# invesalius/invesalius3

Measured on AMD Instinct MI355X. Metric: Mvoxel/s segmentation + Mtriangles/s marching-cubes, 512^3 int16, 1/2/4/8 GPU, higher is better.
Workload: dtype i16; 1 GPU; configs[1]: 512x512x512 int16 per GPU, threshold(226..3071) + 26-neighbour region-grow + marching-cubes(mask@127); global_voxels=134217728, parallelism=z-slab x1, collectives=none, overlap=none

## Files before the change

include/ivx.h:

```cpp
#ifndef IVX_H
#define IVX_H
#include <stddef.h>
#include <stdint.h>

#ifdef __cplusplus
extern "C" {
#endif

#define IVX_OK 0
#define IVX_EINVAL (-1)
#define IVX_ERANGE (-2)
#define IVX_ENOMEM (-3)
#define IVX_EDOM (-4)
#define IVX_EHIP (-5)
#define IVX_ESTALE (-6)

#define IVX_U8 0
#define IVX_I16 1
#define IVX_F64 2
#define IVX_U16 3
#define IVX_F32 4
#define IVX_I32 5
#define IVX_I64 6
#define IVX_I8 7
// ... 307 lines not shown

int ivx_mask_snapshot_header_bytes(int64_t n, size_t *nbytes);
int ivx_dev_mask_snapshot_scan(const uint8_t *src, int64_t n, void *header, int64_t *literal_blocks, void *stream);
int ivx_dev_mask_snapshot_pack(const uint8_t *src, int64_t n, const void *header, void *pool, int64_t literal_blocks, void *stream);
int ivx_dev_mask_snapshot_restore(uint8_t *dst, int64_t n, const void *header, const void *pool, int64_t literal_blocks,
                                  int64_t plane_bytes, uint8_t *plane_flags, void *stream);
int ivx_mask_snapshot(const uint8_t *matrix, size_t nbytes, void **header, void **pool, int64_t *literal_blocks);
int ivx_mask_snapshot_restore(uint8_t *matrix, size_t nbytes, const void *header, const void *pool, int64_t literal_blocks,
                              size_t plane_bytes, int64_t *planes_written);

int ivx_dev_mask_boolean(int op, const uint8_t *m1, const uint8_t *m2, uint8_t *out, int64_t n, void *stream);
int ivx_dev_masked_density_i16(const int16_t *img, const uint8_t *mask, int64_t n, void *acc5, void *stream);
int ivx_mask_boolean(int op, const uint8_t *m1, const int64_t st1[3], const uint8_t *m2, const int64_t st2[3], uint8_t *out,
                     const int64_t sto[3], const int64_t shape[3]);
int ivx_masked_density_i16(const int16_t *img, const int64_t img_strides[3], const uint8_t *mask,
                           const int64_t mask_strides[3], const int64_t shape[3], double *out5);

int ivx_dev_convolve_non_zero(const double *volume, int64_t sz, int64_t sy, int64_t sx, const double *kernel, int64_t skz,
                              int64_t sky, int64_t skx, int cval, double *out, void *stream);
int ivx_mask_area_scratch_bytes(int64_t sz, int64_t sy, int64_t sx, size_t *nbytes);
int ivx_dev_mask_area_u8(const uint8_t *mask, int64_t sz, int64_t sy, int64_t sx, const double *kernel27_dev,
                         double *scratch, double *area_dev, void *stream);
int ivx_convolve_non_zero(const double *volume, const int64_t shape[3], const int64_t vol_strides[3], const double *kernel,
                          const int64_t kshape[3], int cval, double *out);
int ivx_mask_area(const uint8_t *mask, const int64_t shape[3], const int64_t mask_strides[3], const double spacing_xyz[3],
                  double *area);

typedef struct ivx_flood_plan {
    int64_t dz, dy, dx;
    int64_t wx;
    uint32_t strct_bits;
} ivx_flood_plan;
int ivx_flood_bits_bytes(const ivx_flood_plan *p, size_t *nbytes);
int ivx_flood_scratch_bytes(const ivx_flood_plan *p, size_t *nbytes);
int ivx_flood_strct_bits(const uint8_t *strct, const int64_t sshape[3], uint32_t *bits);
int ivx_dev_flood_clear(const ivx_flood_plan *p, uint64_t *reached, void *scratch, void *stream);
int ivx_dev_flood_candidates(const ivx_flood_plan *p, int dtype, const void *data, double t0, double t1,
                             const uint8_t *barrier, int barrier_mode, double fill, uint64_t *cand, void *stream);
int ivx_dev_flood_candidates_ranges(const ivx_flood_plan *p, const int16_t *data, double t0, double t1,
                                    const uint8_t *barrier, int barrier_mode, double fill, const uint32_t *ranges,
                                    uint64_t *cand, void *stream);
int ivx_dev_flood_seed(const ivx_flood_plan *p, int dtype, const void *data, double t0, double t1,
                       const int64_t *seeds_xyz, int64_t nseeds, uint64_t *cand, uint64_t *reached,
                       void *scratch, void *stream);
int ivx_dev_flood_run(const ivx_flood_plan *p, const uint64_t *cand, uint64_t *reached, void *scratch,
                      int *rounds, void *stream);
int ivx_dev_flood_grow(const ivx_flood_plan *p, int dtype, const void *data, double t0, double t1,
                       const int64_t *seeds_xyz, int64_t nseeds, uint64_t *cand, uint64_t *reached, void *scratch,
                       int *rounds, void *stream);
int ivx_dev_flood_visits(const ivx_flood_plan *p, const void *scratch, uint32_t out[2], void *stream);
int ivx_flood_describe(const ivx_flood_plan *p, int64_t nseeds, int32_t out[8]);
int ivx_dev_flood_arm_gate(const void *scratch, uint32_t *word, uint32_t value, uint32_t below_tiles);
int ivx_dev_flood_disarm_gate(const void *scratch);
int ivx_dev_gate_wait(const uint32_t *word, uint32_t value, uint32_t timeout_us, void *stream);
int ivx_dev_gate_open(uint32_t *word, uint32_t value, void *stream);
int ivx_dev_flood_mark_slab(const ivx_flood_plan *p, void *scratch, int64_t z0, int64_t z1, void *stream);
int ivx_dev_bits_combine(uint64_t *dst, const uint64_t *src, int64_t nwords, int op, void *stream);
int ivx_dev_flood_or_plane(const ivx_flood_plan *p, const uint64_t *cand, uint64_t *reached, int64_t z,
                           const uint64_t *plane, void *scratch, int *changed, void *stream);
int ivx_dev_flood_or_planes(const ivx_flood_plan *p, const uint64_t *cand, uint64_t *reached, int64_t z_a,
                            const uint64_t *plane_a, int64_t z_b, const uint64_t *plane_b, void *scratch, int *changed,
                            void *stream);
int ivx_dev_flood_or_planes_dev(const ivx_flood_plan *p, const uint64_t *cand, uint64_t *reached, int64_t z_a,
                                const uint64_t *plane_a, int64_t z_b, const uint64_t *plane_b, void *scratch,
                                uint32_t *changed_dev, void *stream);
int ivx_dev_flood_or_planes_acc(const ivx_flood_plan *p, const uint64_t *cand, uint64_t *reached, int64_t z_a,
                                const uint64_t *plane_a, int64_t z_b, const uint64_t *plane_b, void *scratch,
                                uint32_t *changed_dev, void *stream);
int ivx_dev_flood_apply(const ivx_flood_plan *p, const uint64_t *reached, int dtype, void *target,
                        double fill, void *stream);
int ivx_dev_flood_apply_levels(const ivx_flood_plan *p, const uint64_t *reached, const uint64_t *inside_bits, uint8_t *mask,
                               int v_in, int v_sel, void *stream);
int ivx_dev_mask_from_planes(const ivx_flood_plan *p, const uint64_t *inside_bits, const uint64_t *reached, uint8_t *mask,
                             int v_in, int v_sel, void *stream);
enum { IVX_FLOOD_WRITE_NONE = 0, IVX_FLOOD_WRITE_MASK_FROM_PLANES = 1, IVX_FLOOD_WRITE_APPLY_LEVELS = 2, IVX_FLOOD_WRITE_APPLY_U8 = 3 };
typedef struct ivx_flood_write {
    int32_t kind, v_in, v_sel, reserved;
    const uint64_t *inside_bits;
    uint8_t *mask;
} ivx_flood_write;
int ivx_dev_flood_grow_select(const ivx_flood_plan *p, int dtype, const void *data, double t0, double t1,
                              const int64_t *seeds_xyz, int64_t nseeds, uint64_t *cand, uint64_t *reached, void *scratch,
                              int *rounds, const ivx_flood_write *write, int look_ahead, void *stream);
int ivx_flood_look_ahead(int64_t n_list, int32_t *look_ahead);
int ivx_dev_flood_apply2(const ivx_flood_plan *p, const uint64_t *reached, uint8_t *out, int fill, uint8_t *mask,
                         int select, void *stream);
int ivx_dev_flood_count(const ivx_flood_plan *p, const uint64_t *reached, int64_t *count, void *stream);
int ivx_flood_edges_bytes(const ivx_flood_plan *p, size_t *nbytes);
int ivx_dev_flood_edges_auto(const ivx_flood_plan *p, const int16_t *data, const uint8_t *out, float pfrac, int fill,
                             uint64_t *edges, void *stream);
int ivx_dev_flood_seed_forced(const ivx_flood_plan *p, const int64_t *seeds_xyz, int64_t nseeds, uint64_t *cand,
                              uint64_t *reached, void *scratch, void *stream);
int ivx_dev_flood_run_edges(const ivx_flood_plan *p, const uint64_t *edges, uint64_t *reached, void *scratch, int *rounds,
                            void *stream);
int ivx_floodfill(int dtype, const void *data, const int64_t shape[3], const int64_t strides[3], int64_t x, int64_t y,
                  int64_t z, double v, int fill, uint8_t *out, const int64_t out_strides[3]);
int ivx_floodfill_auto_threshold(const int16_t *data, const int64_t shape[3], const int64_t strides[3],
                                 const int64_t *seeds_xyz, int64_t nseeds, float pfrac, int fill, uint8_t *out,
                                 const int64_t out_strides[3]);
int ivx_dev_jump_flooding(float *dist, int32_t *owners, const int64_t shape[3], const int32_t *sites_host, int64_t nsites,
                          int normalize, void *stream);
int ivx_jump_flooding(float *dist, const int64_t dist_strides[3], int32_t *owners, const int64_t owner_strides[3],
                      const int64_t shape[3], const int32_t *sites, int64_t nsites, int normalize);
int ivx_floodfill_threshold(int dtype, const void *data, const int64_t shape[3], const int64_t strides[3],
                            const int64_t *seeds_xyz, int64_t nseeds, double t0, double t1, int fill,
                            const uint8_t *strct, const int64_t sshape[3], uint8_t *out,
                            const int64_t out_strides[3]);
int ivx_floodfill_threshold_inplace(int dtype, void *data, const int64_t shape[3], const int64_t strides[3],
                                    const int64_t *seeds_xyz, int64_t nseeds, double t0, double t1,
                                    double fill, const uint8_t *strct, const int64_t sshape[3]);

int ivx_dev_fill_holes(uint8_t *mask, const uint32_t *labels, int64_t n, uint32_t nlabels, uint32_t max_size,
                       uint32_t *sizes , int *status2 ,
                       void *stream);
int ivx_fill_holes_automatically(uint8_t *mask, const int64_t shape[3], const int64_t mask_strides[3],
                                 const uint32_t *labels, const int64_t label_strides[3], uint32_t nlabels,
                                 uint32_t max_size, int *modified);
int ivx_dev_fill_holes_auto(uint8_t *mask, int64_t dz, int64_t dy, int64_t dx, const uint8_t *strct, const int64_t sshape[3],
                            uint32_t max_size, int *modified, void *stream);
int ivx_fill_holes_auto(uint8_t *mask, const int64_t shape[3], const int64_t mask_strides[3], const uint8_t *strct,
                        const int64_t sshape[3], uint32_t max_size, int *modified);

int ivx_dev_lut_u16(const int16_t *img, int64_t n, double window, double level, int top255, uint16_t *out,
                    void *stream);
int ivx_dev_lut_i16(const int16_t *img, int64_t n, double window, double level, int top255, int16_t *out,
                    void *stream);
int ivx_dev_shift_min_u16(const int16_t *img, int64_t n, int imin, uint16_t *out, void *stream);
int ivx_dev_morph_gradient_u16(const uint16_t *in, int64_t dz, int64_t dy, int64_t dx, const int size[3],
                               uint16_t *out, void *stream);
int ivx_dev_watershed_merge(uint8_t *mask, const uint8_t *tmp, int64_t n, int overwrite, void *stream);
int ivx_watershed_prepare(const int16_t *img, const int64_t shape[3], const int64_t strides[3], int use_ww_wl,
                          double window, double level, const int gradient_size[3] , uint16_t *out);
int ivx_watershed_merge(uint8_t *mask, const int64_t shape[3], const int64_t mask_strides[3], const uint8_t *tmp,
                        const int64_t tmp_strides[3], int overwrite);

int ivx_dev_sk_cost_levels(const uint16_t *image, int mdtype, const void *markers, int64_t dz, int64_t dy, int64_t dx,
                           const uint8_t strct[27], uint16_t *C, int max_levels, double stop_frac, int *levels_done,
                           int64_t *reached, int64_t *rounds, void *stream);
int ivx_dev_ws_cost_levels(const uint16_t *cost_image, int mdtype, const void *markers, int64_t dz, int64_t dy, int64_t dx,
                           uint16_t *C, int max_levels, double stop_frac, int *levels_done, int64_t *reached,
                           int64_t *rounds, void *stream);
int ivx_dev_watershed_ift(const uint16_t *cost, int mdtype, const void *markers, int64_t dz, int64_t dy, int64_t dx,
                          const uint8_t strct[27], void *out_labels ,
                          uint8_t *out_u8 , uint16_t *cost_out , int64_t stats[16],
                          void *stream);
int ivx_watershed_ift(int idtype , const void *input, const int64_t shape[3], int mdtype,
                      const void *markers, const uint8_t strct[27], void *output, uint16_t *cost_out, int64_t stats[16]);

int ivx_dev_watershed_sk(const uint16_t *image, int mdtype, const void *markers, int64_t dz, int64_t dy, int64_t dx,
                         const uint8_t strct[27], void *out_labels ,
                         int32_t *out_i32 , uint8_t *out_u8 ,
                         uint16_t *cost_out , int64_t stats[16], void *stream);
int ivx_watershed_sk(int idtype , const void *input, const int64_t shape[3], int mdtype,
                     const void *markers, const uint8_t strct[27], int32_t *output, uint16_t *cost_out, int64_t stats[16]);

int ivx_do_watershed(const int16_t *img, const int64_t shape[3], const int64_t strides[3], int mdtype, const void *markers,
                     const uint8_t strct[27], int algorithm, const int gradient_size[3] ,
                     int use_ww_wl, double window, double level, uint8_t *out_u8, int64_t stats[16]);
int ivx_do_watershed_into(const int16_t *img, const int64_t shape[3], const int64_t strides[3], int mk_src_dtype, const void *markers,
                          const int64_t mk_strides[3], int mdtype, const uint8_t strct[27], int algorithm,
                          const int gradient_size[3] , int use_ww_wl, double window, double level,
                          uint8_t *out_u8, const int64_t out_strides[3], int64_t stats[16]);

int ivx_dev_masked_stats_i16(const int16_t *img, const uint8_t *sel, int64_t n, int64_t out3[3], void *stream);
int ivx_dev_or_equal_u8(uint8_t *dst, const uint8_t *src, int64_t n, int value, void *stream);
int ivx_dev_flood_apply_where(uint8_t *dst, const uint8_t *src, int64_t n, int value, int fill, void *stream);
// ... 190 lines not shown
```

invesalius3_amd/_lib.py:

```python
from __future__ import annotations

import ctypes
import os

import numpy as np

_HERE = os.path.dirname(os.path.abspath(__file__))
LIB_PATH = os.environ.get("IVX_LIB_PATH") or os.path.join(_HERE, "libivx.so")

IVX_OK, IVX_EINVAL, IVX_ERANGE, IVX_ENOMEM, IVX_EDOM, IVX_EHIP, IVX_ESTALE = 0, -1, -2, -3, -4, -5, -6
U8, I16, F64, U16, F32, I32, I64, I8 = 0, 1, 2, 3, 4, 5, 6, 7
DT = {np.dtype(np.uint8): U8, np.dtype(np.int16): I16, np.dtype(np.float64): F64, np.dtype(np.uint16): U16, np.dtype(np.float32): F32, np.dtype(np.int32): I32,
      np.dtype(np.int64): I64}
MIP_MAX, MIP_MIN, MIP_MEAN, MIP_SUM = 0, 1, 2, 3

c_i64 = ctypes.c_int64
c_vp = ctypes.c_void_p


class McParams(ctypes.Structure):
    _fields_ = [
        ("dtype", ctypes.c_int32), ("pad_xy", ctypes.c_int32), ("pad_bottom", ctypes.c_int32),
        ("pad_top", ctypes.c_int32), ("vtk_pz", ctypes.c_int32), ("niso", ctypes.c_int32),
        ("nz", c_i64), ("ny", c_i64), ("nx", c_i64), ("roi_start", c_i64),
        ("pad_value", ctypes.c_double), ("spacing", ctypes.c_double * 3), ("iso", ctypes.c_double * 2),
    ]


class FloodPlan(ctypes.Structure):
    _fields_ = [("dz", c_i64), ("dy", c_i64), ("dx", c_i64), ("wx", c_i64), ("strct_bits", ctypes.c_uint32)]


FLOOD_WRITE_NONE, FLOOD_WRITE_MASK_FROM_PLANES, FLOOD_WRITE_APPLY_LEVELS, FLOOD_WRITE_APPLY_U8 = 0, 1, 2, 3


class FloodWrite(ctypes.Structure):
    _fields_ = [("kind", ctypes.c_int32), ("v_in", ctypes.c_int32), ("v_sel", ctypes.c_int32), ("reserved", ctypes.c_int32),
                ("inside_bits", c_vp), ("mask", c_vp)]


class VolrenParams(ctypes.Structure):
    _fields_ = [
        ("width", ctypes.c_int32), ("height", ctypes.c_int32), ("mip", ctypes.c_int32), ("shade", ctypes.c_int32),
        ("skip", ctypes.c_int32), ("n_table", ctypes.c_int32), ("out_u8", ctypes.c_int32), ("clip", ctypes.c_int32),
        ("origin", ctypes.c_double * 3), ("du", ctypes.c_double * 3), ("dv", ctypes.c_double * 3),
        ("dir", ctypes.c_double * 3), ("spacing", ctypes.c_double * 3), ("dt", ctypes.c_double),
        ("ambient", ctypes.c_double), ("diffuse", ctypes.c_double), ("specular", ctypes.c_double),
        ("specular_power", ctypes.c_double), ("background", ctypes.c_double * 3), ("clip_normal", ctypes.c_double * 3),
        ("clip_origin", ctypes.c_double * 3),
    ]


ROI_ELLIPSE, ROI_POLYGON, ROI_MAX_POINTS, ROI_RECORD_BYTES = 0, 1, 2048, 40


class Roi(ctypes.Structure):
    _fields_ = [
        ("image", c_vp), ("row_stride", c_i64), ("elem_stride", c_i64), ("h", c_i64), ("w", c_i64),
        ("kind", ctypes.c_int32), ("n_points", ctypes.c_int32), ("first_point", c_i64),
        ("sx", ctypes.c_double), ("sy", ctypes.c_double), ("cx", ctypes.c_double), ("cy", ctypes.c_double),
        ("a2", ctypes.c_double), ("b2", ctypes.c_double),
        ("x0", c_i64), ("y0", c_i64), ("x1", c_i64), ("y1", c_i64), ("first_block", c_i64), ("n_blocks", c_i64),
    ]


class StaleError(RuntimeError):
    """IVX_ESTALE: a registered host array (resident.bind) was written without a touch; raised only with the stale check on."""


def _declare(lib):
    u64, sz, u64p = ctypes.c_uint64, ctypes.c_size_t, ctypes.POINTER(ctypes.c_uint64)
    i64p = ctypes.POINTER(c_i64)
    for name, args in (("ivx_host_register", [c_vp, sz, u64p]), ("ivx_host_touch", [u64]), ("ivx_host_touch_range", [u64, sz, sz]),
                       ("ivx_host_release", [u64]), ("ivx_host_stats", [u64, u64p]), ("ivx_host_count", [u64p]),
                       ("ivx_host_set_check", [ctypes.c_int]), ("ivx_transfer_stats", [u64p]),
                       ("ivx_upload_strided", [c_vp, c_vp, i64p, i64p, sz]), ("ivx_download_strided", [c_vp, i64p, i64p, c_vp, sz]),
                       ("ivx_image_ranges_bytes", [c_i64, c_i64, c_i64, ctypes.POINTER(sz)]),
                       ("ivx_dev_image_ranges_i16", [c_vp, c_i64, c_i64, c_i64, c_vp, c_vp]),
                       ("ivx_dev_threshold_i16_bits_ranges", [c_vp, c_i64, c_i64, c_i64, ctypes.c_int, ctypes.c_int, c_vp, c_vp, c_vp,
                                                              ctypes.c_int, c_vp]),
                       ("ivx_dev_threshold_i16_plane", [c_vp, c_i64, c_i64, c_i64, ctypes.c_int, ctypes.c_int, c_vp, c_vp]),
                       ("ivx_dev_threshold_i16_plane_ranges", [c_vp, c_i64, c_i64, c_i64, ctypes.c_int, ctypes.c_int, c_vp, c_vp,
                                                               ctypes.c_int, c_vp]),
                       ("ivx_dev_mask_from_planes", [ctypes.POINTER(FloodPlan), c_vp, c_vp, c_vp, ctypes.c_int, ctypes.c_int, c_vp]),
                       ("ivx_dev_flood_candidates_ranges", [ctypes.POINTER(FloodPlan), c_vp, ctypes.c_double, ctypes.c_double, c_vp,
                                                            ctypes.c_int, ctypes.c_double, c_vp, c_vp, c_vp]),
                       ("ivx_dev_flood_grow_select", [ctypes.POINTER(FloodPlan), ctypes.c_int, c_vp, ctypes.c_double, ctypes.c_double,
                                                      c_vp, c_i64, c_vp, c_vp, c_vp, ctypes.POINTER(ctypes.c_int),
                                                      ctypes.POINTER(FloodWrite), ctypes.c_int, c_vp]),
                       ("ivx_flood_look_ahead", [c_i64, ctypes.POINTER(ctypes.c_int32)]),
                       ("ivx_dev_image_flip", [c_vp, c_i64, c_i64, c_i64, sz, ctypes.c_int, c_vp]),
                       ("ivx_image_flip", [c_vp, i64p, i64p, sz, ctypes.c_int]),
                       ("ivx_dev_image_swap_axes", [c_vp, c_i64, c_i64, c_i64, sz, ctypes.c_int, ctypes.c_int, c_vp, c_vp]),
                       ("ivx_image_swap_axes", [c_vp, i64p, i64p, sz, ctypes.c_int, ctypes.c_int, c_vp, i64p]),
                       ("ivx_image_tilt_scratch_bytes", [c_i64, c_i64, c_i64, ctypes.POINTER(sz)]),
                       ("ivx_dev_image_fix_gantry_tilt", [c_vp, c_i64, c_i64, c_i64, c_vp, c_vp, sz, c_vp, c_vp]),
                       ("ivx_image_fix_gantry_tilt", [c_vp, i64p, i64p, c_vp, c_vp]),
                       ("ivx_host_zero", [c_vp, sz]), ("ivx_host_register_zero", [c_vp, sz, u64p]),
                       ("ivx_slice_show_tables_bytes", [ctypes.c_int, ctypes.POINTER(sz)]),
                       ("ivx_dev_slice_show", [c_vp, c_i64, c_i64] * 3 + [c_i64, c_i64, c_vp, c_vp, c_vp, c_vp]),
                       ("ivx_slice_show", [c_vp, c_i64, c_i64] * 3 + [c_i64, c_i64, c_vp, c_vp, c_vp]),
                       ("ivx_mask_snapshot_header_bytes", [c_i64, ctypes.POINTER(sz)]),
                       ("ivx_dev_mask_snapshot_scan", [c_vp, c_i64, c_vp, i64p, c_vp]),
                       ("ivx_dev_mask_snapshot_pack", [c_vp, c_i64, c_vp, c_vp, c_i64, c_vp]),
                       ("ivx_dev_mask_snapshot_restore", [c_vp, c_i64, c_vp, c_vp, c_i64, c_i64, c_vp, c_vp]),
                       ("ivx_mask_snapshot", [c_vp, sz, ctypes.POINTER(c_vp), ctypes.POINTER(c_vp), i64p]),
                       ("ivx_mask_snapshot_restore", [c_vp, sz, c_vp, c_vp, c_i64, sz, i64p]),
                       ("ivx_dev_surface_raster", [c_vp, c_i64, c_vp, c_i64, c_vp, ctypes.c_int, c_vp, c_vp]),
                       ("ivx_dev_surface_resolve", [c_vp, ctypes.c_int, c_vp, ctypes.c_int, c_vp, ctypes.c_int, c_vp, c_vp, c_vp, c_vp]),
                       ("ivx_surface_render", [c_vp, ctypes.c_int, c_vp, ctypes.c_int, c_vp, ctypes.c_int, c_vp, c_vp, c_vp]),
                       ("ivx_dev_roi_density", [c_vp, c_i64, c_vp, c_vp, c_i64, c_vp, c_vp]),
                       ("ivx_roi_density", [c_vp, c_i64, c_vp, c_i64, c_vp]),
                       ("ivx_dev_m3e_filter", [c_i64, c_i64, c_vp, c_vp, c_i64, ctypes.c_int, c_vp, c_vp]),
                       ("ivx_dev_m3e_cut", [c_vp, i64p, i64p, c_vp, ctypes.c_double, c_vp, c_i64, c_i64, c_vp, c_vp, ctypes.c_int, c_vp, c_vp]),
                       ("ivx_dev_m3e_brush_stroke", [c_vp, c_vp, i64p, i64p, c_vp, c_vp, c_vp, c_i64, ctypes.c_double, ctypes.c_int, c_vp,
                                                     c_vp]),
                       ("ivx_dev_m3e_equal", [c_vp, c_vp, c_i64, ctypes.POINTER(ctypes.c_int), c_vp]),
                       ("ivx_dev_m3e_apply", [c_vp, c_vp, i64p, i64p, c_vp, c_vp]),
                       ("ivx_m3e_filter", [c_i64, c_i64, c_vp, c_vp, c_i64, ctypes.c_int, c_vp]),
                       ("ivx_m3e_cut", [c_vp, i64p, i64p, c_vp, ctypes.c_double, c_vp, c_i64, c_i64, c_vp, c_vp, c_i64, c_vp, c_vp,
                                        ctypes.c_int, i64p]),
                       ("ivx_m3e_brush_stroke", [c_vp, c_vp, i64p, i64p, c_vp, c_vp, c_i64, ctypes.c_double, ctypes.c_int, i64p]),
                       ("ivx_m3e_apply", [c_vp, c_vp, i64p, i64p, i64p]), ("ivx_m3e_flag_planes", [c_vp, i64p, i64p])):
        fn = getattr(lib, name)
        fn.argtypes, fn.restype = args, ctypes.c_int


_lib = None


def lib() -> ctypes.CDLL:
    global _lib
    if _lib is None:
        if not os.path.exists(LIB_PATH):
            raise ImportError(
                "libivx.so not found at %s: build it with `python -m invesalius3_amd.build` "
                "(there is no CPU fallback in this package)" % LIB_PATH)
        _lib = ctypes.CDLL(LIB_PATH)
        _lib.ivx_last_error.restype = ctypes.c_char_p
        _declare(_lib)
    return _lib


def last_error() -> str:
    return (lib().ivx_last_error() or b"").decode("utf-8", "replace")


def check(rc: int, what: str = "ivx") -> int:
    if rc >= 0:
        return rc
    msg = "%s: %s" % (what, last_error())
    if rc == IVX_EINVAL:
        raise TypeError(msg)
    if rc == IVX_ERANGE:
        raise IndexError(msg)
    if rc == IVX_ENOMEM:
        raise MemoryError(msg)
    if rc == IVX_EDOM:
        raise ValueError(msg)
    if rc == IVX_ESTALE:
        raise StaleError(msg)
    raise RuntimeError(msg)


def i64(seq):
    return (c_i64 * len(seq))(*[int(v) for v in seq])


def ptr(a: np.ndarray):
    return ctypes.c_void_p(a.ctypes.data)


# ... 60 lines not shown
```

invesalius3_amd/csrc/ivx_internal.h:

```cpp
#pragma once
#include <hip/hip_runtime.h>
#include <stdint.h>
#include <stdio.h>
#include <string.h>

#include "../../include/ivx.h"

namespace ivx {

void set_error(const char *fmt, ...);

#define IVX_HIP(expr)                                                                      \
    do {                                                                                   \
        hipError_t e__ = (expr);                                                           \
        if (e__ != hipSuccess) {                                                           \
            ivx::set_error("%s:%d %s -> %s", __FILE__, __LINE__, #expr, hipGetErrorString(e__)); \
            return e__ == hipErrorOutOfMemory ? IVX_ENOMEM : IVX_EHIP;                     \
        }                                                                                  \
    } while (0)

bool trace_enabled();
#define IVX_LAUNCH_CHECK()                                                                 \
    do {                                                                                   \
        IVX_HIP(hipGetLastError());                                                        \
        if (ivx::trace_enabled()) {                                                        \
            fprintf(stderr, "ivx trace: launched %s:%d ...", __FILE__, __LINE__);          \
            fflush(stderr);                                                                \
            IVX_HIP(hipDeviceSynchronize());                                               \
            fprintf(stderr, " ok\n");                                                      \
        }                                                                                  \
    } while (0)

#define IVX_REQUIRE(cond, code, ...)                                                       \
    do {                                                                                   \
        if (!(cond)) {                                                                     \
            ivx::set_error(__VA_ARGS__);                                                   \
            return (code);                                                                 \
        }                                                                                  \
    } while (0)

static inline hipStream_t S(void *s) { return (hipStream_t)s; }
static inline int64_t cdiv(int64_t a, int64_t b) { return (a + b - 1) / b; }
static inline size_t dtype_size(int dt) {
    switch (dt) {
    case IVX_U8: return 1;
    case IVX_I16: return 2;
    case IVX_U16: return 2;
    case IVX_F64: return 8;
    default: return 0;
    }
}

enum { WS_IN = 0, WS_OUT, WS_AUX0, WS_AUX1, WS_AUX2, WS_AUX3, WS_SMALL, WS_CCL0, WS_CCL1, WS_MCLIST, WS_MCV, WS_MCST, WS_MESH, WS_MESH2, WS_HOLES, WS_LUT, WS_WSIFT, WS_WSSK, WS_WSA, WS_WSLINK, WS_COUNT };
int ws_get(int slot, size_t nbytes, void **dptr);
int ws_get_s(int slot, hipStream_t stream, size_t nbytes, void **dptr);
uint64_t host_epoch();
int ws_release_s(int slot, hipStream_t stream, size_t keep_below);
struct HostCallGuard {
    HostCallGuard();
    ~HostCallGuard();
};
int hs_get(int slot, size_t nbytes, void **hptr);

int copy_h2d(void *dst_dev, const void *src, size_t n);
int copy_d2h(void *dst, const void *src_dev, size_t n);

int upload_strided(void *dst_dev, const void *src, const int64_t shape[3], const int64_t strides[3], size_t isz,
                   int hslot);
int download_strided(void *dst, const int64_t shape[3], const int64_t strides[3], const void *src_dev, size_t isz,
                     int hslot);
int download_strided2(void *dst, const int64_t shape[2], const int64_t strides[2], const void *src_dev, size_t isz,
                      int hslot);
int mirror_host_view(const void *view, const int64_t shape[3], const int64_t strides[3], size_t isz, void *d_scratch, int hslot);

struct MirrorHold;
int mirror_acquire(const void *p, size_t n, bool reads, MirrorHold **hold, void **mirror);
int mirror_fetch(MirrorHold *hold, void *host, const void *mirror, size_t n);
void mirror_release(MirrorHold *hold, size_t written);

void ccl_forget_stream(void *stream);
void ccl_invalidate(const void *scratch);
int ccl_small_components(const ivx_flood_plan *p, const uint64_t *cand, uint64_t *out, uint32_t max_size, int *any_small,
                         const void *scratch_key, hipStream_t st);
bool ccl_supported(uint32_t strct_bits);
int ccl_run(const ivx_flood_plan *p, const uint64_t *cand, uint64_t *reached, const void *scratch_key, hipStream_t st);
enum FloodMode {
    FLOOD_SYMMETRIC,
    FLOOD_DIRECTED,
    FLOOD_LINEAR,
};
int flood_run(const ivx_flood_plan *p, const uint64_t *planes, FloodMode mode, uint64_t *reached, void *scratch, int *rounds,
              void *stream);

int mailbox_publish(const void *dsrc, int ndwords, hipStream_t st, uint32_t *seq_out);
int mailbox_wait(uint32_t seq, hipStream_t st, uint32_t *out, int ndwords);
int mailbox_reserve(uint32_t **slot_out, uint32_t *seq_out);
int mailbox_wait_reserved(uint32_t seq, hipStream_t st, uint32_t *out, int ndwords, int *got);
int vote_publish(int32_t *votes, hipStream_t st, uint32_t *seq_out);
int progress_line(hipStream_t stream, volatile unsigned long long **line, uint32_t *tag);
void progress_forget_stream(void *stream);

}
```

invesalius3_amd/csrc/k_flood.hip:

```cpp
#include <math.h>
#include <map>
#include <mutex>
#include <stdlib.h>

#include "flood_tiles.h"
#include "words_from_records.h"

namespace {

constexpr int NT = TY * TZ;
constexpr int HY = TY + 2, HZ = TZ + 2;
constexpr int BATCH = 8;
constexpr int SUB = 1;
constexpr unsigned int CLOSED = 0x40u;

template <typename T> __device__ __forceinline__ double as_double(T v) { return (double)v; }

template <typename T, int BAR>
__global__ __launch_bounds__(256) void k_flood_candidates16(const short8_t *__restrict__ data,
                                                            const uint4 *__restrict__ bar, int64_t nchunks, double t0,
                                                            double t1, double fill, uint16_t *__restrict__ cand) {
    const int64_t stride = (int64_t)gridDim.x * blockDim.x;
    const int lo = (int)ceil(t0 < -70000.0 ? -70000.0 : t0), hi = (int)floor(t1 > 70000.0 ? 70000.0 : t1);
    const unsigned fb = (unsigned)(uint8_t)fill;
    for (int64_t c = (int64_t)blockIdx.x * blockDim.x + threadIdx.x; c < nchunks; c += stride) {
        const short8_t a = __builtin_nontemporal_load(&data[2 * c]);
        const short8_t b = __builtin_nontemporal_load(&data[2 * c + 1]);
        uint4 q = make_uint4(0, 0, 0, 0);
        if (BAR == 1) q = bar[c];
        const unsigned bw[4] = {q.x, q.y, q.z, q.w};
        unsigned m = 0;
#pragma unroll
        for (int e = 0; e < 16; e++) {
            const int v = (int)(T)(e < 8 ? a[e & 7] : b[e & 7]);
            bool ok = v >= lo && v <= hi;
            if (BAR == 1) ok = ok && ((bw[e >> 2] >> (8 * (e & 3))) & 0xffu) != fb;
            if (BAR == 2) ok = ok && (double)v != fill;
            m |= ok ? (1u << e) : 0u;
        }
        cand[c] = (uint16_t)m;
    }
}

__global__ __launch_bounds__(256) void k_flood_candidates_words(const short8_t *__restrict__ data, const unsigned *__restrict__ ranges,
                                                                int64_t nwords, double t0, double t1,
                                                                unsigned long long *__restrict__ cand) {
    const int lo = (int)ceil(t0 < -70000.0 ? -70000.0 : t0), hi = (int)floor(t1 > 70000.0 ? 70000.0 : t1);
    words_from_records(data, ranges, nwords, lo, hi, cand);
}

__global__ __launch_bounds__(256) void k_flood_candidates16_ranges(const short8_t *__restrict__ data,
                                                                   const uint4 *__restrict__ bar,
                                                                   const unsigned *__restrict__ ranges, int64_t nchunks,
                                                                   double t0, double t1, double fill,
                                                                   uint16_t *__restrict__ cand) {
    const int64_t stride = (int64_t)gridDim.x * blockDim.x;
    const int lo = (int)ceil(t0 < -70000.0 ? -70000.0 : t0), hi = (int)floor(t1 > 70000.0 ? 70000.0 : t1);
    const unsigned fb = (unsigned)(uint8_t)fill;
    int64_t c = (int64_t)blockIdx.x * blockDim.x + threadIdx.x;
    if (c >= nchunks) return;
    unsigned rec = ranges[c >> 2];
    for (;;) {
        const int64_t cn = c + stride;
        unsigned rec_next = 0;
        if (cn < nchunks) rec_next = ranges[cn >> 2];
        const int mn = (int)(short)(rec & 0xffffu), mx = (int)(short)(rec >> 16);
        unsigned m = 0;
        if (!(mx < lo || mn > hi)) {
            const bool inside = mn >= lo && mx <= hi;
            if (inside) {
                m = 0xffffu;
            } else {
                const short8_t a = __builtin_nontemporal_load(&data[2 * c]);
                const short8_t b = __builtin_nontemporal_load(&data[2 * c + 1]);
#pragma unroll
                for (int e = 0; e < 16; e++) {
                    const int v = (int)(e < 8 ? a[e & 7] : b[e & 7]);
                    m |= (v >= lo && v <= hi) ? (1u << e) : 0u;
                }
            }
            if (m) {
                const uint4 q = bar[c];
                const unsigned bw[4] = {q.x, q.y, q.z, q.w};
#pragma unroll
                for (int e = 0; e < 16; e++)
                    if (((bw[e >> 2] >> (8 * (e & 3))) & 0xffu) == fb) m &= ~(1u << e);
            }
        }
        cand[c] = (uint16_t)m;
// ... 813 lines not shown
                if (!ok[d]) continue;
                const int64_t n = base + x + off[d];
                const int nv = data[n];
                if (out[n] != fill && nv >= t0 && nv <= t1) m[d] |= 1u << e;
            }
        }
        const int64_t plane = total;
#pragma unroll
        for (int d = 0; d < 6; d++) edges[d * plane + i] = (uint8_t)m[d];
    }
}

__global__ void k_flood_seed_forced(Tiles t, const int64_t *__restrict__ seeds, int64_t nseeds,
                                    unsigned long long *__restrict__ cand, unsigned long long *__restrict__ reached,
                                    uint8_t *__restrict__ dirty) {
    const int64_t n = (int64_t)blockIdx.x * blockDim.x + threadIdx.x;
    if (n >= nseeds) return;
    const int64_t x = seeds[3 * n], y = seeds[3 * n + 1], z = seeds[3 * n + 2];
    const int64_t w = (z * t.dy + y) * t.wx + (x >> 6);
    const unsigned long long bit = 1ull << (x & 63);
    if (cand) atomicOr(&cand[w], bit);
    atomicOr(&reached[w], bit);
    mark_tile_nbhd(t, dirty, z / TZ, y / TY, x >> 6);
}

template <typename T>
__global__ __launch_bounds__(256) void k_flood_apply(Tiles t, const uint8_t *__restrict__ reached, T *__restrict__ out,
                                                     T fill) {
    const int64_t bpr = t.wx * 8;
    const int64_t total = t.dz * t.dy * bpr;
    const int64_t stride = (int64_t)gridDim.x * blockDim.x;
    const bool aligned8 = ((uintptr_t)out & 7) == 0 && (t.dx & 7) == 0;
    for (int64_t i = (int64_t)blockIdx.x * blockDim.x + threadIdx.x; i < total; i += stride) {
        const unsigned m = reached[i];
        if (!m) continue;
        const int64_t row = i / bpr, q = i - row * bpr;
        T *o = out + row * t.dx + q * 8;
        if (sizeof(T) == 1 && m == 0xffu && aligned8) {
            *reinterpret_cast<unsigned long long *>(o) = 0x0101010101010101ull * (unsigned long long)(uint8_t)fill;
            continue;
        }
#pragma unroll
        for (int e = 0; e < 8; e++)
            if (m >> e & 1u) o[e] = fill;
    }
}

__global__ __launch_bounds__(256) void k_flood_apply16(const uint16_t *__restrict__ reached, int64_t nchunks,
                                                       uint4 *__restrict__ out, uint8_t fill) {
    const int64_t stride = (int64_t)gridDim.x * 1024;
    const unsigned int f4 = 0x01010101u * fill;
    for (int64_t i0 = (int64_t)blockIdx.x * 1024 + threadIdx.x; i0 < nchunks; i0 += stride) {
        unsigned int m[4];
        uint4 o[4];
#pragma unroll
        for (int u = 0; u < 4; u++) {
            const int64_t i = i0 + u * 256;
            m[u] = i < nchunks ? reached[i] : 0u;
            o[u] = make_uint4(0u, 0u, 0u, 0u);
        }
#pragma unroll
        for (int u = 0; u < 4; u++)
            if (m[u] && m[u] != 0xffffu) o[u] = out[i0 + u * 256];
#pragma unroll
        for (int u = 0; u < 4; u++) {
            if (!m[u]) continue;
            uint4 v = make_uint4(f4, f4, f4, f4);
            if (m[u] != 0xffffu) {
                auto blend = [&](unsigned int old, unsigned int bits4) {
                    const unsigned int sel = ((bits4 & 1u) * 0xffu) | ((bits4 >> 1 & 1u) * 0xff00u) |
                                             ((bits4 >> 2 & 1u) * 0xff0000u) | ((bits4 >> 3 & 1u) * 0xff000000u);
                    return (old & ~sel) | (f4 & sel);
                };
                v.x = blend(o[u].x, m[u] & 15u);
                v.y = blend(o[u].y, m[u] >> 4 & 15u);
                v.z = blend(o[u].z, m[u] >> 8 & 15u);
                v.w = blend(o[u].w, m[u] >> 12 & 15u);
            }
            out[i0 + u * 256] = v;
        }
    }
}

struct ApplyWhen {
    const unsigned int *next_len;
    unsigned long long *line;
    unsigned long long report;
};
template <bool ALL>
__global__ __launch_bounds__(256) void k_flood_apply_levels16(const uint16_t *__restrict__ reached, const uint16_t *__restrict__ inside,
                                                              int64_t nchunks, uint4 *__restrict__ out, uint8_t v_in, uint8_t v_sel,
                                                              ApplyWhen when) {
    if (when.next_len) {
        if (*when.next_len != 0u) return;
        if (blockIdx.x == 0 && threadIdx.x == 0) __hip_atomic_store(&when.line[2], when.report, __ATOMIC_RELAXED, __HIP_MEMORY_SCOPE_SYSTEM);
    }
    const int64_t stride = (int64_t)gridDim.x * 1024;
    const unsigned int in4 = 0x01010101u * v_in, sel4 = 0x01010101u * v_sel;
    for (int64_t i0 = (int64_t)blockIdx.x * 1024 + threadIdx.x; i0 < nchunks; i0 += stride) {
        unsigned int m[4], b[4];
#pragma unroll
        for (int u = 0; u < 4; u++) {
            const int64_t i = i0 + u * 256;
            m[u] = i < nchunks && (!ALL || reached) ? reached[i] : 0u;
            b[u] = i < nchunks ? inside[i] : 0u;
        }
#pragma unroll
        for (int u = 0; u < 4; u++) {
            if (ALL ? i0 + u * 256 >= nchunks : !m[u]) continue;
            auto bytes = [](unsigned int bits4) { return ((bits4 * 0x00204081u) & 0x01010101u) * 0xffu; };
            auto word = [&](unsigned int r4, unsigned int i4) {
                const unsigned int rs = bytes(r4);
                return (sel4 & rs) | (in4 & bytes(i4) & ~rs);
            };
            out[i0 + u * 256] = make_uint4(word(m[u] & 15u, b[u] & 15u), word(m[u] >> 4 & 15u, b[u] >> 4 & 15u),
                                           word(m[u] >> 8 & 15u, b[u] >> 8 & 15u), word(m[u] >> 12 & 15u, b[u] >> 12 & 15u));
        }
    }
}

__global__ __launch_bounds__(256) void k_flood_apply2(Tiles t, const uint8_t *__restrict__ reached, uint8_t *__restrict__ out,
                                                      uint8_t fill, uint8_t *__restrict__ mask, uint8_t select) {
    const int64_t bpr = t.wx * 8;
    const int64_t total = t.dz * t.dy * bpr;
    const int64_t stride = (int64_t)gridDim.x * blockDim.x;
    const bool aligned8 = (((uintptr_t)out | (uintptr_t)mask) & 7) == 0;
    for (int64_t i = (int64_t)blockIdx.x * blockDim.x + threadIdx.x; i < total; i += stride) {
        const unsigned m = reached[i];
        if (!m) continue;
        const int64_t row = i / bpr, q = i - row * bpr;
        const int64_t base = row * t.dx + q * 8;
        if (m == 0xffu && ((t.dx & 7) == 0) && aligned8) {
            *reinterpret_cast<unsigned long long *>(out + base) = 0x0101010101010101ull * fill;
            *reinterpret_cast<unsigned long long *>(mask + base) = 0x0101010101010101ull * select;
            continue;
        }
#pragma unroll
        for (int e = 0; e < 8; e++)
            if (m >> e & 1u) {
                out[base + e] = fill;
                mask[base + e] = select;
            }
    }
}

__global__ __launch_bounds__(256) void k_flood_count(const unsigned long long *__restrict__ bits, int64_t nwords,
                                                     unsigned long long *__restrict__ total) {
    unsigned long long s = 0;
    const int64_t stride = (int64_t)gridDim.x * blockDim.x;
    for (int64_t i = (int64_t)blockIdx.x * blockDim.x + threadIdx.x; i < nwords; i += stride) s += __popcll(bits[i]);
#pragma unroll
    for (int o = 32; o > 0; o >>= 1) s += __shfl_xor(s, o, 64);
    if ((threadIdx.x & 63) == 0 && s) atomicAdd(total, s);
}

static inline int grid_for(int64_t n) {
    const int64_t b = ivx::cdiv(n, 256);
    return (int)(b < 1 ? 1 : (b < 32768 ? b : 32768));
}

template <typename T>
static int run_candidates(const Tiles &t, const void *data, double t0, double t1, const uint8_t *bar, int bar_mode,
                          double fill, uint8_t *cand, hipStream_t st) {
    const int64_t total = t.dz * t.dy * t.wx * 8;
    if (!total) return IVX_OK;
    if (sizeof(T) == 2 && t.dx % 64 == 0 && (((uintptr_t)data | (uintptr_t)bar | (uintptr_t)cand) & 15) == 0) {
        const int64_t nchunks = t.dz * t.dy * t.dx / 16;
        const int64_t blocks = ivx::cdiv(nchunks, 256);
        const int gg = (int)(blocks < 16384 ? blocks : 16384);
        const short8_t *d8 = (const short8_t *)data;
        const uint4 *b4 = (const uint4 *)bar;
        uint16_t *c16 = (uint16_t *)cand;
        if (bar_mode == 0) hipLaunchKernelGGL((k_flood_candidates16<T, 0>), dim3(gg), dim3(256), 0, st, d8, b4, nchunks, t0, t1, fill, c16);
        else if (bar_mode == 1) hipLaunchKernelGGL((k_flood_candidates16<T, 1>), dim3(gg), dim3(256), 0, st, d8, b4, nchunks, t0, t1, fill, c16);
        else hipLaunchKernelGGL((k_flood_candidates16<T, 2>), dim3(gg), dim3(256), 0, st, d8, b4, nchunks, t0, t1, fill, c16);
        IVX_LAUNCH_CHECK();
        return IVX_OK;
    }
    const int g = grid_for(total);
    if (bar_mode == 0)
        hipLaunchKernelGGL((k_flood_candidates<T, 0>), dim3(g), dim3(256), 0, st, (const T *)data, bar, t, t0, t1, fill, cand);
    else if (bar_mode == 1)
        hipLaunchKernelGGL((k_flood_candidates<T, 1>), dim3(g), dim3(256), 0, st, (const T *)data, bar, t, t0, t1, fill, cand);
    else
        hipLaunchKernelGGL((k_flood_candidates<T, 2>), dim3(g), dim3(256), 0, st, (const T *)data, bar, t, t0, t1, fill, cand);
    IVX_LAUNCH_CHECK();
    return IVX_OK;
}

}

extern "C" int ivx_flood_bits_bytes(const ivx_flood_plan *p, size_t *nbytes) {
    Tiles t;
    int rc = make_tiles(p, &t);
    if (rc) return rc;
    *nbytes = al256((size_t)(t.dz * t.dy * t.wx) * 8);
    return IVX_OK;
}

extern "C" int ivx_flood_scratch_bytes(const ivx_flood_plan *p, size_t *nbytes) {
// ... 183 lines not shown
        return e && !strcmp(e, "ccl");
    }();
    return ccl;
}
static bool coarse_ok(const Tiles &t, ivx::FloodMode mode) {
    static const bool coarse_on = [] {
        const char *e = getenv("IVX_FLOOD_COARSE");
        return !(e && e[0] == '0');
    }();
    return coarse_on && mode == ivx::FLOOD_SYMMETRIC && t.conn != 0 && t.wx <= 64 && (t.nty + 2) * (t.ntz + 2) <= CROWS_MAX &&
           t.nty * t.ntz <= (int64_t)CT * CRP;
}
static Blocks coarse_blocks(const Tiles &t) {
    static const int bxs_env = [] {
        const char *e = getenv("IVX_FLOOD_BLOCK");
        return e ? atoi(e) : 0;
    }();
    Blocks bk;
    bk.bxs = 16;
    while (bk.bxs < 64 && ((64 / bk.bxs) * t.wx > 64 || bk.bxs < bxs_env)) bk.bxs *= 2;
    bk.q = 64 / bk.bxs;
    return bk;
}
static int coarse_lanes(const Tiles &t) {
    int ct = 64;
    while (ct < CT && ct < t.nty * t.ntz) ct *= 2;
    return ct;
}
template <bool FRESH>
static int coarse_pass(const Tiles &t, const FScratch &s, char *scr, const uint64_t *cand, uint64_t *reached, const Fresh &f,
                       int ncnt, hipStream_t st) {
    const Blocks bk = coarse_blocks(t);
    uint8_t *dirty0 = (uint8_t *)(scr + s.off_dirty0), *dirty1 = (uint8_t *)(scr + s.off_dirty1);
    unsigned int *cnt = (unsigned int *)(scr + s.off_cnt), *list0 = (unsigned int *)(scr + s.off_list0);
    unsigned long long *rowF = (unsigned long long *)(scr + s.off_full), *rowW = (unsigned long long *)(scr + s.off_whole);
    unsigned int *seed_ok = (unsigned int *)(scr + s.off_status) + 8;
    const unsigned groups = (unsigned)(t.nty * t.ntz);
    const int ct = coarse_lanes(t);
    hipLaunchKernelGGL(k_flood_block_flags<FRESH>, dim3(groups), dim3(256), 0, st, t, bk, (unsigned long long *)cand,
                       (const unsigned long long *)reached, dirty0, dirty1, rowF, rowW, cnt, ncnt, f.sp, f.dtype, f.data, f.t0,
                       f.t1, seed_ok);
    IVX_LAUNCH_CHECK();
    auto coarse = t.conn == 26 ? k_flood_coarse<26, FRESH> : t.conn == 18 ? k_flood_coarse<18, FRESH> : k_flood_coarse<6, FRESH>;
    hipLaunchKernelGGL(coarse, dim3(1), dim3(ct), 0, st, t, bk, (const unsigned long long *)rowF, rowW, f.sp,
                       (const unsigned int *)seed_ok);
    IVX_LAUNCH_CHECK();
    hipLaunchKernelGGL(k_flood_block_apply<FRESH>, dim3(groups), dim3(256), 0, st, t, bk, (const unsigned long long *)cand,
                       (unsigned long long *)reached, (const unsigned long long *)rowW, dirty0, list0, cnt, f.sp,
                       (const unsigned int *)seed_ok);
    IVX_LAUNCH_CHECK();
    return IVX_OK;
}
static unsigned round_grid_cap(const Tiles &t) { return (unsigned)(t.ntiles < 1536 ? t.ntiles : 1536); }
template <typename Done>
static int poll_line(volatile unsigned long long *line, long spins, hipStream_t st, Done done, const char *never,
                     unsigned long long *word) {
    for (long n = 0; n < spins; n++) {
        *word = __atomic_load_n((const unsigned long long *)line, __ATOMIC_ACQUIRE);
        if (done(*word)) return IVX_OK;
#if defined(__x86_64__)
        __builtin_ia32_pause();
#endif
    }
    IVX_HIP(hipStreamSynchronize(st));
    *word = __atomic_load_n((const unsigned long long *)line, __ATOMIC_ACQUIRE);
    IVX_REQUIRE(done(*word), IVX_EHIP, "%s", never);
    return IVX_OK;
}
static int levels_check(const Tiles &t, const uint64_t *reached, const uint64_t *inside_bits, const uint8_t *mask, int v_in, int v_sel,
                        bool all) {
    if (all) {
        IVX_REQUIRE(inside_bits && mask, IVX_EINVAL, "mask_from_planes: null plane or mask");
        IVX_REQUIRE(t.dx % 64 == 0 && ((uintptr_t)mask & 15) == 0 && (((uintptr_t)inside_bits | (uintptr_t)reached) & 7) == 0, IVX_EINVAL,
                    "mask_from_planes: rows of whole 64-voxel words, a 16-byte aligned mask and 8-byte aligned planes only");
        IVX_REQUIRE(v_in >= 0 && v_in <= 255 && v_sel >= 0 && v_sel <= 255, IVX_EINVAL, "mask_from_planes: levels are bytes");
    } else {
        IVX_REQUIRE(reached && inside_bits && mask, IVX_EINVAL, "flood_apply_levels: null plane or mask");
        IVX_REQUIRE(t.dx % 64 == 0 && ((uintptr_t)mask & 15) == 0, IVX_EINVAL,
                    "flood_apply_levels: rows of whole 64-voxel words and a 16-byte aligned mask only");
        IVX_REQUIRE(v_in >= 0 && v_in <= 255 && v_sel >= 0 && v_sel <= 255, IVX_EINVAL, "flood_apply_levels: levels are bytes");
    }
    return IVX_OK;
}
static int launch_levels(const Tiles &t, const uint64_t *reached, const uint64_t *inside, uint8_t *mask, int v_in, int v_sel, bool all,
                         const ApplyWhen &when, hipStream_t st) {
    const int64_t nchunks = t.dz * t.dy * t.dx / 16;
    if (!nchunks) return IVX_OK;
    const int64_t blocks = ivx::cdiv(nchunks, 1024);
    auto k = all ? k_flood_apply_levels16<true> : k_flood_apply_levels16<false>;
    hipLaunchKernelGGL(k, dim3((unsigned)(blocks < 16384 ? blocks : 16384)), dim3(256), 0, st, (const uint16_t *)reached,
                       (const uint16_t *)inside, nchunks, (uint4 *)mask, (uint8_t)v_in, (uint8_t)v_sel, when);
    IVX_LAUNCH_CHECK();
    return IVX_OK;
}
constexpr unsigned AHEAD_LONG_LIST = 384u;
static int default_look_ahead(unsigned n_list) { return n_list >= AHEAD_LONG_LIST ? 0 : 1; }
struct EarlyWrite {
    const ivx_flood_write *w;
    bool written;
};
constexpr unsigned EARLY_BELOW = 96u;
constexpr int EARLY_TRIES = 2;
static int flood_run_impl(const ivx_flood_plan *p, const uint64_t *cand, ivx::FloodMode mode, uint64_t *reached, void *scratch_,
                          int *rounds, void *stream, const Fresh *fresh = nullptr, int look_ahead = -1, EarlyWrite *early = nullptr) {
    const bool sym = mode == ivx::FLOOD_SYMMETRIC;
    Tiles t;
    int rc = make_tiles(p, &t);
    if (rc) return rc;
    if (rounds) *rounds = 0;
    hipStream_t st = ivx::S(stream);
    GateArm arm = {nullptr, 0u, 0u};
    {
        std::lock_guard<std::mutex> lk(g_gates_mu);
        auto it = g_gates.find(scratch_);
        if (it != g_gates.end()) {
            arm = it->second;
            g_gates.erase(it);
        }
    }
    struct GateGuard {
        GateArm &a;
        hipStream_t st;
        ~GateGuard() {
            if (a.word) hipLaunchKernelGGL(k_gate_set, dim3(1), dim3(64), 0, st, a.word, a.value);
        }
    } gate_guard = {arm, st};
    if (t.ntiles == 0) return IVX_OK;
    const FScratch s = make_fscratch(t);
    char *scr = (char *)scratch_;
    uint8_t *dirty[2] = {(uint8_t *)(scr + s.off_dirty0), (uint8_t *)(scr + s.off_dirty1)};
    unsigned int *cnt = (unsigned int *)(scr + s.off_cnt);
    constexpr int CCL_ESCAPE_ROUNDS = 48;
    if (sym && flood_mode_ccl() && ivx::ccl_supported(p->strct_bits)) {
        if (rounds) *rounds = 1;
        IVX_HIP(hipMemsetAsync(dirty[0], 0, (size_t)t.ntiles, st));
        return ivx::ccl_run(p, cand, reached, scratch_, st);
    }
    int total_rounds = 0;
    unsigned int *list[2] = {(unsigned int *)(scr + s.off_list0), (unsigned int *)(scr + s.off_list1)};
    constexpr int RING = 2 * BATCH;
    static const int env_ahead = [] {
        const char *e = getenv("IVX_FLOOD_BATCH");
        if (!e || !*e) return -1;
        const int v = atoi(e);
        return v < 0 ? 0 : (v > BATCH ? BATCH : v);
    }();
    const int fixed_ahead = env_ahead >= 0 ? env_ahead : (look_ahead > BATCH ? BATCH : look_ahead);
    int ahead = fixed_ahead >= 0 ? fixed_ahead : 1;
    if (coarse_ok(t, mode)) {
        static const Fresh no_seeds = {0, nullptr, 0.0, 0.0, {{}, 0}};
        rc = fresh ? coarse_pass<true>(t, s, scr, cand, reached, *fresh, CNT_CLEARED, st)
                   : coarse_pass<false>(t, s, scr, cand, reached, no_seeds, CNT_CLEARED, st);
        if (rc) return rc;
    } else {
        IVX_REQUIRE(!fresh, IVX_EINVAL, "flood: the fused start needs the coarse pass");
        IVX_HIP(hipMemsetAsync(cnt, 0, CNT_CLEARED * 4, st));
        hipLaunchKernelGGL(k_flood_build_list, dim3((unsigned)ivx::cdiv(t.ntiles, 256)), dim3(256), 0, st, t, dirty[0], list[0], cnt);
        IVX_LAUNCH_CHECK();
    }
    volatile unsigned long long *line = nullptr;
    uint32_t tag = 0;
    if ((rc = ivx::progress_line(st, &line, &tag))) return rc;
    const unsigned grid_max = round_grid_cap(t);
    unsigned grid = grid_max;
    int64_t queued = 0;
    auto round_kernel = mode == ivx::FLOOD_LINEAR ? k_flood_round_list<2> : mode == ivx::FLOOD_DIRECTED ? k_flood_round_list<1> : k_flood_round_list<0>;
    auto queue_round = [&]() -> int {
        const int r = (int)(queued % RING), cur = (int)(queued & 1);
        const unsigned int tr = (unsigned int)(tag << 24) | (unsigned int)((queued + 1) & 0xffffff);
        hipLaunchKernelGGL(round_kernel, dim3(grid), dim3(NT), 0, st, t, (const unsigned long long *)cand,
                           (unsigned long long *)reached, (const unsigned int *)list[cur], (const unsigned int *)(cnt + r), dirty[cur],
                           dirty[cur ^ 1], list[cur ^ 1], cnt + (r + 1) % RING, cnt + (r + 2) % RING, cnt,
                           (unsigned long long *)line, tr,
                           arm.word, arm.value, arm.below);
        IVX_LAUNCH_CHECK();
        queued++;
        return IVX_OK;
    };
    static const bool trace = getenv("IVX_FLOOD_TRACE") != nullptr;
    static const bool early_on = [] {
        const char *e = getenv("IVX_FLOOD_EARLY");
        return !(e && e[0] == '0');
    }();
    const bool early_all = early && early->w->kind == IVX_FLOOD_WRITE_MASK_FROM_PLANES;
    int early_left = 0;
    if (early_on && early && (early_all || early->w->kind == IVX_FLOOD_WRITE_APPLY_LEVELS) &&
        levels_check(t, reached, early->w->inside_bits, early->w->mask, early->w->v_in, early->w->v_sel, early_all) == IVX_OK)
        early_left = EARLY_TRIES;
    if (early_left) __atomic_store_n((unsigned long long *)line + 2, 0ull, __ATOMIC_RELEASE);
    int64_t early_at = -1;
    unsigned long long early_report = 0;
    bool early_seen = false;
    unsigned int prev_list = 0xffffffffu;
    int64_t seen = 0;
    for (;;) {
        while (queued < seen + 1 + ahead)
            if ((rc = queue_round())) return rc;
        unsigned long long v = 0;
        rc = poll_line(line, 20000000L, st,
                       [&](unsigned long long w) {
                           if (early_at >= 0 && __atomic_load_n((const unsigned long long *)line + 2, __ATOMIC_ACQUIRE) == early_report)
                               return early_seen = true;
                           return (uint32_t)(w >> 56) == tag && (int64_t)((w >> 32) & 0xffffffull) > seen;
                       },
                       "flood: the queued rounds never reported", &v);
        if (rc) return rc;
        if (early_seen) {
            const unsigned long long u = __atomic_load_n((const unsigned long long *)line + 1, __ATOMIC_ACQUIRE);
            total_rounds = (uint32_t)(u >> 56) == tag ? (int)((u >> 32) & 0xffffffull) : 0;
            early->written = true;
            if (trace) fprintf(stderr, "ivx flood: the write behind round %lld went ahead (%d rounds with work)\n", (long long)early_at, total_rounds);
            break;
        }
        seen = (int64_t)((v >> 32) & 0xffffffull);
        const unsigned int n_list = (unsigned int)(v & 0xffffffffull);
        if (trace) fprintf(stderr, "ivx flood: round %lld starts with %u of %lld tiles (%lld queued)\n", (long long)seen, n_list,
                           (long long)t.ntiles, (long long)queued);
        if (n_list < arm.below) arm.word = nullptr;
        grid = n_list >= 384u ? grid_max : (n_list >= 96u ? (grid_max < 512u ? grid_max : 512u) : (grid_max < 128u ? grid_max : 128u));
        if (fixed_ahead < 0) ahead = default_look_ahead(n_list);
        if (n_list == 0) {
            const unsigned long long u = __atomic_load_n((const unsigned long long *)line + 1, __ATOMIC_ACQUIRE);
            total_rounds = (uint32_t)(u >> 56) == tag ? (int)((u >> 32) & 0xffffffull) : 0;
            if (early_at >= 0 && total_rounds <= early_at) early->written = true;
            break;
        }
        if (early_at >= 0 && seen > early_at) early_at = -1;
        if (early_left > 0 && early_at < 0 && n_list < EARLY_BELOW && n_list <= prev_list / 2u) {
            early_at = queued;
            early_left--;
            early_report = ((unsigned long long)tag << 56) | ((unsigned long long)(queued & 0xffffff) << 32) | 1ull;
            if (trace) fprintf(stderr, "ivx flood: write queued behind round %lld\n", (long long)queued);
            rc = launch_levels(t, reached, early->w->inside_bits, early->w->mask, early->w->v_in, early->w->v_sel, early_all,
                               ApplyWhen{cnt + queued % RING, (unsigned long long *)line, early_report}, st);
            if (rc) return rc;
        }
        prev_list = n_list;
        total_rounds = (int)seen;
        if (sym && total_rounds >= CCL_ESCAPE_ROUNDS && ivx::ccl_supported(p->strct_bits)) {
            IVX_HIP(hipMemsetAsync(dirty[0], 0, (size_t)t.ntiles, st));
            IVX_HIP(hipMemsetAsync(dirty[1], 0, (size_t)t.ntiles, st));
            if ((rc = ivx::ccl_run(p, cand, reached, scratch_, st))) return rc;
            total_rounds += 1;
            break;
        }
        IVX_REQUIRE(total_rounds < (1 << 24) - 64, IVX_EHIP, "flood: did not converge");
    }
    if (rounds) *rounds = total_rounds;
    return IVX_OK;
}

constexpr int AHEAD_CHAINED = 3;
int ivx::flood_run(const ivx_flood_plan *p, const uint64_t *planes, ivx::FloodMode mode, uint64_t *reached, void *scratch,
                   int *rounds, void *stream) {
    return flood_run_impl(p, planes, mode, reached, scratch, rounds, stream, nullptr, AHEAD_CHAINED);
}

extern "C" int ivx_dev_flood_run(const ivx_flood_plan *p, const uint64_t *cand, uint64_t *reached, void *scratch_,
                                 int *rounds, void *stream) {
    return flood_run_impl(p, cand, ivx::FLOOD_SYMMETRIC, reached, scratch_, rounds, stream, nullptr, AHEAD_CHAINED);
}
static bool fused_start(const Tiles &t, int64_t nseeds) {
    static const bool fused_on = [] {
        const char *e = getenv("IVX_FLOOD_FUSED");
        return !(e && e[0] == '0');
    }();
    return fused_on && nseeds >= 1 && nseeds <= 16 && t.ntiles > 0 && !flood_mode_ccl() && coarse_ok(t, ivx::FLOOD_SYMMETRIC);
}
static int flood_grow_impl(const ivx_flood_plan *p, int dtype, const void *data, double t0, double t1, const int64_t *seeds_xyz,
                           int64_t nseeds, uint64_t *cand, uint64_t *reached, void *scratch_, int *rounds, void *stream,
                           int look_ahead, EarlyWrite *early = nullptr) {
    Tiles t;
    int rc = make_tiles(p, &t);
    if (rc) return rc;
    IVX_REQUIRE(ivx::dtype_size(dtype), IVX_EINVAL, "flood: unsupported dtype %d", dtype);
    for (int64_t n = 0; n < nseeds; n++) {
        const int64_t x = seeds_xyz[3 * n], y = seeds_xyz[3 * n + 1], z = seeds_xyz[3 * n + 2];
        IVX_REQUIRE(x >= 0 && y >= 0 && z >= 0 && x < t.dx && y < t.dy && z < t.dz, IVX_ERANGE,
                    "flood: seed (%lld,%lld,%lld) outside volume (%lld,%lld,%lld) [x,y,z]", (long long)x, (long long)y,
                    (long long)z, (long long)t.dx, (long long)t.dy, (long long)t.dz);
    }
    if (!fused_start(t, nseeds)) {
        if ((rc = ivx_dev_flood_clear(p, reached, scratch_, stream))) return rc;
        if ((rc = ivx_dev_flood_seed(p, dtype, data, t0, t1, seeds_xyz, nseeds, cand, reached, scratch_, stream))) return rc;
        return flood_run_impl(p, cand, ivx::FLOOD_SYMMETRIC, reached, scratch_, rounds, stream, nullptr, look_ahead, early);
    }
    ivx::ccl_invalidate(scratch_);
    Fresh f;
    f.dtype = dtype;
    f.data = data;
    f.t0 = t0;
    f.t1 = t1;
    f.sp.n = (int)nseeds;
    for (int64_t n = 0; n < nseeds; n++)
        for (int q = 0; q < 3; q++) f.sp.xyz[n][q] = seeds_xyz[3 * n + q];
    return flood_run_impl(p, cand, ivx::FLOOD_SYMMETRIC, reached, scratch_, rounds, stream, &f, look_ahead, early);
}
extern "C" int ivx_dev_flood_grow(const ivx_flood_plan *p, int dtype, const void *data, double t0, double t1,
                                  const int64_t *seeds_xyz, int64_t nseeds, uint64_t *cand, uint64_t *reached, void *scratch_,
                                  int *rounds, void *stream) {
    return flood_grow_impl(p, dtype, data, t0, t1, seeds_xyz, nseeds, cand, reached, scratch_, rounds, stream, AHEAD_CHAINED);
}
extern "C" int ivx_flood_look_ahead(int64_t n_list, int32_t *look_ahead) {
    IVX_REQUIRE(look_ahead && n_list >= 0, IVX_EINVAL, "flood_look_ahead: NULL or negative argument");
    *look_ahead = default_look_ahead(n_list > 0xffffffffll ? 0xffffffffu : (unsigned)n_list);
    return IVX_OK;
}
extern "C" int ivx_dev_flood_visits(const ivx_flood_plan *p, const void *scratch_, uint32_t out[2], void *stream) {
    IVX_REQUIRE(scratch_ && out, IVX_EINVAL, "flood_visits: NULL argument");
    Tiles t;
    int rc = make_tiles(p, &t);
    if (rc) return rc;
    out[0] = out[1] = 0u;
    if (t.ntiles == 0) return IVX_OK;
    const FScratch s = make_fscratch(t);
    hipStream_t st = ivx::S(stream);
    unsigned int w[CNT_CLEARED - STATS_AT];
    IVX_HIP(hipMemcpyAsync(w, (const char *)scratch_ + s.off_cnt + STATS_AT * 4, sizeof w, hipMemcpyDeviceToHost, st));
    IVX_HIP(hipStreamSynchronize(st));
    out[0] = w[0];
    for (int k = 0; k < HIST; k++) out[0] += w[HIST_AT - STATS_AT + k];
    out[1] = w[HIST_AT - STATS_AT];
    return IVX_OK;
}
extern "C" int ivx_flood_describe(const ivx_flood_plan *p, int64_t nseeds, int32_t out[8]) {
    IVX_REQUIRE(out, IVX_EINVAL, "flood_describe: NULL argument");
// ... 78 lines not shown
    return IVX_OK;
}
extern "C" int ivx_dev_flood_disarm_gate(const void *scratch) {
    std::lock_guard<std::mutex> lk(g_gates_mu);
    g_gates.erase(scratch);
    return IVX_OK;
}
extern "C" int ivx_dev_gate_open(uint32_t *word, uint32_t value, void *stream) {
    IVX_REQUIRE(word, IVX_EINVAL, "gate_open: NULL argument");
    hipLaunchKernelGGL(k_gate_set, dim3(1), dim3(64), 0, ivx::S(stream), word, value);
    IVX_LAUNCH_CHECK();
    return IVX_OK;
}
extern "C" int ivx_dev_gate_wait(const uint32_t *word, uint32_t value, uint32_t timeout_us, void *stream) {
    IVX_REQUIRE(word, IVX_EINVAL, "gate_wait: NULL argument");
    hipLaunchKernelGGL(k_gate_wait, dim3(1), dim3(64), 0, ivx::S(stream), word, value, (unsigned long long)timeout_us * 100ull);
    IVX_LAUNCH_CHECK();
    return IVX_OK;
}

extern "C" int ivx_dev_flood_mark_slab(const ivx_flood_plan *p, void *scratch_, int64_t z0, int64_t z1, void *stream) {
    Tiles t;
    int rc = make_tiles(p, &t);
    if (rc) return rc;
    if (z0 < 0) z0 = 0;
    if (z1 > t.dz) z1 = t.dz;
    if (z1 <= z0 || t.ntiles == 0) return IVX_OK;
    const FScratch s = make_fscratch(t);
    const int64_t tz0 = z0 / TZ, tz1 = ivx::cdiv(z1, TZ);
    const int64_t n = (tz1 - tz0) * t.nty * t.wx;
    hipLaunchKernelGGL(k_flood_mark, dim3((unsigned)ivx::cdiv(n, 256)), dim3(256), 0, ivx::S(stream), t, tz0, tz1,
                       (uint8_t *)((char *)scratch_ + s.off_dirty0));
    IVX_LAUNCH_CHECK();
    return IVX_OK;
}

extern "C" int ivx_dev_flood_apply(const ivx_flood_plan *p, const uint64_t *reached, int dtype, void *target,
                                   double fill, void *stream) {
    Tiles t;
    int rc = make_tiles(p, &t);
    if (rc) return rc;
    const int64_t total = t.dz * t.dy * t.wx * 8;
    if (!total) return IVX_OK;
    const int g = grid_for(total);
    hipStream_t st = ivx::S(stream);
    const uint8_t *r = (const uint8_t *)reached;
    if (dtype == IVX_U8 && t.dx % 64 == 0 && ((uintptr_t)target & 15) == 0) {
        const int64_t nchunks = t.dz * t.dy * t.dx / 16;
        const int64_t blocks = ivx::cdiv(nchunks, 1024);
        hipLaunchKernelGGL(k_flood_apply16, dim3((unsigned)(blocks < 16384 ? blocks : 16384)), dim3(256), 0, st,
                           (const uint16_t *)reached, nchunks, (uint4 *)target, (uint8_t)fill);
        IVX_LAUNCH_CHECK();
        return IVX_OK;
    }
    switch (dtype) {
    case IVX_U8: hipLaunchKernelGGL(k_flood_apply<uint8_t>, dim3(g), dim3(256), 0, st, t, r, (uint8_t *)target, (uint8_t)fill); break;
    case IVX_I16: hipLaunchKernelGGL(k_flood_apply<int16_t>, dim3(g), dim3(256), 0, st, t, r, (int16_t *)target, (int16_t)fill); break;
    case IVX_U16: hipLaunchKernelGGL(k_flood_apply<uint16_t>, dim3(g), dim3(256), 0, st, t, r, (uint16_t *)target, (uint16_t)fill); break;
    case IVX_F64: hipLaunchKernelGGL(k_flood_apply<double>, dim3(g), dim3(256), 0, st, t, r, (double *)target, fill); break;
    default: ivx::set_error("flood: unsupported dtype %d", dtype); return IVX_EINVAL;
    }
    IVX_LAUNCH_CHECK();
    return IVX_OK;
}

extern "C" int ivx_dev_flood_apply_levels(const ivx_flood_plan *p, const uint64_t *reached, const uint64_t *inside_bits, uint8_t *mask,
                                          int v_in, int v_sel, void *stream) {
    Tiles t;
    int rc = make_tiles(p, &t);
    if (rc) return rc;
    if ((rc = levels_check(t, reached, inside_bits, mask, v_in, v_sel, false))) return rc;
    return launch_levels(t, reached, inside_bits, mask, v_in, v_sel, false, ApplyWhen{nullptr, nullptr, 0ull}, ivx::S(stream));
}

extern "C" int ivx_dev_mask_from_planes(const ivx_flood_plan *p, const uint64_t *inside_bits, const uint64_t *reached, uint8_t *mask,
                                        int v_in, int v_sel, void *stream) {
    Tiles t;
    int rc = make_tiles(p, &t);
    if (rc) return rc;
    if ((rc = levels_check(t, reached, inside_bits, mask, v_in, v_sel, true))) return rc;
    return launch_levels(t, reached, inside_bits, mask, v_in, v_sel, true, ApplyWhen{nullptr, nullptr, 0ull}, ivx::S(stream));
}

extern "C" int ivx_dev_flood_grow_select(const ivx_flood_plan *p, int dtype, const void *data, double t0, double t1,
                                         const int64_t *seeds_xyz, int64_t nseeds, uint64_t *cand, uint64_t *reached,
                                         void *scratch_, int *rounds, const ivx_flood_write *write, int look_ahead, void *stream) {
    IVX_REQUIRE(write && write->kind >= IVX_FLOOD_WRITE_NONE && write->kind <= IVX_FLOOD_WRITE_APPLY_U8, IVX_EINVAL,
                "flood_grow_select: no write description, or one of an unknown kind");
    IVX_REQUIRE(write->kind == IVX_FLOOD_WRITE_NONE || write->mask, IVX_EINVAL, "flood_grow_select: the write has no mask");
    EarlyWrite early = {write, false};
    int rc = flood_grow_impl(p, dtype, data, t0, t1, seeds_xyz, nseeds, cand, reached, scratch_, rounds, stream, look_ahead, &early);
    if (rc || early.written) return rc;
    switch (write->kind) {
    case IVX_FLOOD_WRITE_MASK_FROM_PLANES:
        return ivx_dev_mask_from_planes(p, write->inside_bits, reached, write->mask, write->v_in, write->v_sel, stream);
    case IVX_FLOOD_WRITE_APPLY_LEVELS:
        return ivx_dev_flood_apply_levels(p, reached, write->inside_bits, write->mask, write->v_in, write->v_sel, stream);
    case IVX_FLOOD_WRITE_APPLY_U8: return ivx_dev_flood_apply(p, reached, IVX_U8, write->mask, (double)write->v_sel, stream);
    default: return IVX_OK;
    }
}

extern "C" int ivx_dev_flood_apply2(const ivx_flood_plan *p, const uint64_t *reached, uint8_t *out, int fill,
                                    uint8_t *mask, int select, void *stream) {
    Tiles t;
    int rc = make_tiles(p, &t);
    if (rc) return rc;
    const int64_t total = t.dz * t.dy * t.wx * 8;
    if (!total) return IVX_OK;
    hipLaunchKernelGGL(k_flood_apply2, dim3(grid_for(total)), dim3(256), 0, ivx::S(stream), t, (const uint8_t *)reached, out,
                       (uint8_t)fill, mask, (uint8_t)select);
    IVX_LAUNCH_CHECK();
    return IVX_OK;
}

extern "C" int ivx_dev_flood_count(const ivx_flood_plan *p, const uint64_t *reached, int64_t *count, void *stream) {
    Tiles t;
    int rc = make_tiles(p, &t);
    if (rc) return rc;
    *count = 0;
    const int64_t nw = t.dz * t.dy * t.wx;
    if (!nw) return IVX_OK;
    void *d_tot;
    if ((rc = ivx::ws_get_s(ivx::WS_SMALL, ivx::S(stream), 64, &d_tot))) return rc;
    hipStream_t st = ivx::S(stream);
    IVX_HIP(hipMemsetAsync(d_tot, 0, 8, st));
    hipLaunchKernelGGL(k_flood_count, dim3(grid_for(nw)), dim3(256), 0, st, (const unsigned long long *)reached, nw,
                       (unsigned long long *)d_tot);
    IVX_LAUNCH_CHECK();
    unsigned long long h = 0;
    IVX_HIP(hipMemcpyAsync(&h, d_tot, 8, hipMemcpyDeviceToHost, st));
    IVX_HIP(hipStreamSynchronize(st));
    *count = (int64_t)h;
    return IVX_OK;
}

template <bool MARK>
__global__ __launch_bounds__(256) void k_flood_or_plane(unsigned long long *__restrict__ dst,
                                                        const unsigned long long *__restrict__ src,
                                                        const unsigned long long *__restrict__ cand, int64_t nwords,
                                                        unsigned int *__restrict__ changed, Tiles t, int64_t z,
                                                        uint8_t *__restrict__ dirty) {
    const int64_t i = (int64_t)blockIdx.x * blockDim.x + threadIdx.x;
    if (i >= nwords) return;
    const unsigned long long add = src[i] & cand[i] & ~dst[i];
    if (add) {
        dst[i] |= add;
        atomicAdd(changed, 1u);
        if (MARK) {
            const int64_t y = i / t.wx, txi = i - y * t.wx;
            mark_tile_nbhd(t, dirty, z / TZ, y / TY, txi);
        }
    }
}

__global__ __launch_bounds__(256) void k_bits_combine(unsigned long long *__restrict__ dst,
                                                      const unsigned long long *__restrict__ src, int64_t n, int op) {
    const int64_t stride = (int64_t)gridDim.x * blockDim.x;
    for (int64_t i = (int64_t)blockIdx.x * blockDim.x + threadIdx.x; i < n; i += stride)
        dst[i] = op == 0 ? (dst[i] | src[i]) : (dst[i] & ~src[i]);
}
extern "C" int ivx_dev_bits_combine(uint64_t *dst, const uint64_t *src, int64_t nwords, int op, void *stream) {
    IVX_REQUIRE(nwords >= 0 && (op == 0 || op == 1), IVX_EINVAL, "bits_combine: bad arguments");
    if (nwords == 0) return IVX_OK;
    const int64_t blocks = ivx::cdiv(nwords, 256);
    hipLaunchKernelGGL(k_bits_combine, dim3((unsigned)(blocks < 8192 ? blocks : 8192)), dim3(256), 0, ivx::S(stream),
                       (unsigned long long *)dst, (const unsigned long long *)src, nwords, op);
    IVX_LAUNCH_CHECK();
    return IVX_OK;
}

extern "C" int ivx_dev_flood_or_plane(const ivx_flood_plan *p, const uint64_t *cand, uint64_t *reached, int64_t z,
                                      const uint64_t *plane, void *scratch_, int *changed, void *stream) {
    Tiles t;
    int rc = make_tiles(p, &t);
    if (rc) return rc;
    IVX_REQUIRE(z >= 0 && z < t.dz, IVX_ERANGE, "flood: plane %lld outside slab", (long long)z);
    const FScratch s = make_fscratch(t);
    const int64_t nw = t.dy * t.wx;
    *changed = 0;
    if (!nw) return IVX_OK;
    hipStream_t st = ivx::S(stream);
    unsigned int *d_chg = (unsigned int *)((char *)scratch_ + s.off_status);
// ... 223 lines not shown
```

invesalius3_amd/csrc/k_mc.hip:

```cpp
#include <algorithm>

#include "mc_common.h"

#define MC_TABLE_QUAL static __device__ __attribute__((aligned(16))) const
#include "../../include/ivx_mc_tables.h"

typedef short short8_t __attribute__((ext_vector_type(8)));
typedef unsigned char uchar16_t __attribute__((ext_vector_type(16)));

using namespace ivx;

namespace {

template <typename T, int NISO>
__global__ __launch_bounds__(256) void k_mc_bits(const T *__restrict__ a, int64_t nrows_src, int64_t nx, int64_t ws,
                                                 double iso0, double iso1, uint8_t *__restrict__ bits0,
                                                 uint8_t *__restrict__ bits1) {
    constexpr int V = 16 / sizeof(T);
    constexpr int OB = V / 8;
    const int64_t cpr = ws * 64 / V;
    const int64_t total = nrows_src * cpr;
    const int64_t stride = (int64_t)gridDim.x * blockDim.x;
    const bool vec = (nx % V == 0) && (((uintptr_t)a & 15) == 0);
    if (vec && ws * 64 == nx) {
        const int64_t nchunk = nrows_src * (nx / V);
        typedef T vec_t __attribute__((ext_vector_type(V)));
        const vec_t *src = reinterpret_cast<const vec_t *>(a);
        for (int64_t t0 = ((int64_t)blockIdx.x * blockDim.x) * 4 + threadIdx.x; t0 < nchunk; t0 += stride * 4) {
            vec_t x[4];
#pragma unroll
            for (int u = 0; u < 4; u++) {
                const int64_t t = t0 + (int64_t)u * blockDim.x;
                if (t < nchunk) x[u] = __builtin_nontemporal_load(&src[t]);
            }
#pragma unroll
            for (int u = 0; u < 4; u++) {
                const int64_t t = t0 + (int64_t)u * blockDim.x;
                if (t >= nchunk) continue;
                unsigned m0 = 0, m1 = 0;
#pragma unroll
                for (int e = 0; e < V; e++) {
                    const double d = (double)(T)x[u][e];
                    m0 |= d >= iso0 ? (1u << e) : 0u;
                    if (NISO == 2) m1 |= d >= iso1 ? (1u << e) : 0u;
                }
                if (OB == 1) {
                    bits0[t] = (uint8_t)m0;
                    if (NISO == 2) bits1[t] = (uint8_t)m1;
                } else {
                    reinterpret_cast<uint16_t *>(bits0)[t] = (uint16_t)m0;
                    if (NISO == 2) reinterpret_cast<uint16_t *>(bits1)[t] = (uint16_t)m1;
                }
            }
        }
        return;
    }
    for (int64_t t = (int64_t)blockIdx.x * blockDim.x + threadIdx.x; t < total; t += stride) {
        const int64_t row = t / cpr, q = t - row * cpr;
        const int64_t x0 = q * V;
        unsigned m0 = 0, m1 = 0;
        if (x0 < nx) {
            const T *r = a + row * nx + x0;
            T v[V];
            if (vec) {
                if (sizeof(T) == 2) {
                    const short8_t c = *reinterpret_cast<const short8_t *>(r);
#pragma unroll
                    for (int e = 0; e < V; e++) v[e] = (T)c[e % 8];
                } else {
                    const uchar16_t c = *reinterpret_cast<const uchar16_t *>(r);
#pragma unroll
                    for (int e = 0; e < V; e++) v[e] = (T)c[e % 16];
                }
            } else {
#pragma unroll
                for (int e = 0; e < V; e++) v[e] = (x0 + e < nx) ? r[e] : (T)0;
            }
#pragma unroll
            for (int e = 0; e < V; e++) {
                const bool valid = vec || (x0 + e < nx);
                const double d = (double)v[e];
                m0 |= (valid && d >= iso0) ? (1u << e) : 0u;
                if (NISO == 2) m1 |= (valid && d >= iso1) ? (1u << e) : 0u;
            }
// ... 32 lines not shown
    const uint64_t exist = mc_lowbits(NX32 - w32 * 64);
    uint64_t srcm = exist;
    if (g.pxy && w32 == 0) srcm &= ~1ull;
    srcm &= mc_lowbits(g.pxy + nx32 - w32 * 64);
    const int32_t x1 = (w32 + 1) * 64;
    const bool exist1 = x1 < NX32;
    const bool src1 = x1 - g.pxy < nx32;
    const int32_t wc = w32 >= ws32 ? (ws32 > 0 ? ws32 - 1 : 0) : w32;
    const int32_t wm = w32 - 1 >= ws32 ? (ws32 > 0 ? ws32 - 1 : 0) : (w32 - 1 < 0 ? 0 : w32 - 1);
    const int32_t wp = w32 + 1 >= ws32 ? (ws32 > 0 ? ws32 - 1 : 0) : w32 + 1;
    const int32_t ja0 = ((int32_t)g.NY - 1 - (int32_t)j) - g.pxy, ka0 = (int32_t)k - g.pb;
    const bool inner = ja0 - 1 >= 0 && ja0 < (int32_t)g.ny && ka0 >= 0 && ka0 + 1 < (int32_t)g.nz;
    if (__all(inner)) {
        const uint64_t padlo = pbits & exist & ~srcm;
        const bool use1 = exist1 && src1;
        const uint32_t nbpad = exist1 ? (uint32_t)pbits & 1u : 0u;
        const uint64_t *row = bits + (uint64_t)((uint32_t)ka0 * (uint32_t)g.ny + (uint32_t)ja0) * (uint64_t)(uint32_t)ws32;
        const uint64_t *pc = row + wc, *pa = row + (g.pxy ? wm : wp);
        const int64_t dj = -g.ws, dk = g.ny * g.ws;
        uint64_t a0[4], a1[4];
#pragma unroll
        for (int q = 0; q < 4; q++) {
            const int64_t d = ((q & 1) ? dj : 0) + ((q >> 1) ? dk : 0);
            a0[q] = pc[d];
            a1[q] = pa[d];
        }
#pragma unroll
        for (int q = 0; q < 4; q++) {
            uint64_t v0;
            uint32_t raw1;
            if (g.pxy) {
                v0 = mc_shl1(a0[q], (uint32_t)(a1[q] >> 32));
                raw1 = (uint32_t)(a0[q] >> 63);
            } else {
                v0 = a0[q];
                raw1 = (uint32_t)a1[q] & 1u;
            }
            const uint64_t lo = (v0 & srcm) | padlo;
            r.c[2 * q] = lo;
            r.c[2 * q + 1] = mc_shr1(lo, use1 ? raw1 : nbpad);
        }
    } else {
        const bool has_m = w32 - 1 >= 0 && w32 - 1 < ws32, has_c = w32 < ws32, has_p = w32 + 1 < ws32;
        uint64_t a0[4], a1[4];
        bool rin[4];
#pragma unroll
        for (int q = 0; q < 4; q++) {
            const int64_t ja = (g.NY - 1 - (j + (q & 1))) - g.pxy, ka = k + (q >> 1) - g.pb;
            rin[q] = ja >= 0 && ja < g.ny && ka >= 0 && ka < g.nz;
            const uint64_t *row = bits + (clampi(ka, g.nz) * g.ny + clampi(ja, g.ny)) * g.ws;
            a0[q] = row[wc];
            a1[q] = g.pxy ? row[wm] : row[wp];
        }
#pragma unroll
        for (int q = 0; q < 4; q++) {
            const uint64_t sc = (rin[q] && has_c) ? a0[q] : 0ull;
            uint64_t v0, raw1;
            if (g.pxy) {
                const uint64_t sm = (rin[q] && has_m) ? a1[q] : 0ull;
                v0 = (sc << 1) | (sm >> 63);
                raw1 = sc >> 63;
            } else {
                const uint64_t sp = (rin[q] && has_p) ? a1[q] : 0ull;
                v0 = sc;
                raw1 = sp & 1ull;
            }
            const uint64_t src = rin[q] ? srcm : 0ull;
            const uint64_t lo = (v0 & src) | (pbits & exist & ~src);
            const uint64_t nb = exist1 ? ((rin[q] && src1) ? raw1 : (pbits & 1ull)) : 0ull;
            r.c[2 * q] = lo;
            r.c[2 * q + 1] = (lo >> 1) | (nb << 63);
        }
    }
    uint64_t any = 0, all = ~0ull;
#pragma unroll
    for (int c = 0; c < 8; c++) {
        any |= r.c[c];
        all &= r.c[c];
    }
    r.active = any & ~all & mc_lowbits(NX32 - 1 - w32 * 64);
    return r;
}

__global__ __launch_bounds__(256) void k_mc_count(const uint64_t *__restrict__ bits, Geom g, size_t nwords,
                                                  uint64_t pbits, uint16_t *__restrict__ counts,
                                                  uint32_t *__restrict__ bsum) {
    __shared__ uint32_t s_part[4], s_wcnt[4];
    __shared__ uint8_t s_ntri[256];
    __shared__ uint64_t s_c[256][5];
    __shared__ uint8_t s_hi[256];
    __shared__ uint16_t s_slot[256];
    const int tid = threadIdx.x, lane = tid & 63, wv = tid >> 6;
    const uint8_t ntri = MC_NTRI[tid];
    const size_t wid = (size_t)blockIdx.x * 256 + tid;
    uint64_t act = 0;
    Corner8 r;
    if (wid < nwords) {
        uint32_t k, j, w;
        mc_split_wid(g, (uint32_t)wid, k, j, w);
        r = load_corners(bits, g, (int64_t)k, (int64_t)j, (int64_t)w, pbits);
        act = r.active;
        if (!act) counts[wid] = 0;
    }
    const unsigned long long am = __ballot(act != 0);
    if (lane == 0) s_wcnt[wv] = (uint32_t)__popcll(am);
    s_ntri[tid] = ntri;
    __syncthreads();
    uint32_t before = 0;
    for (int q = 0; q < wv; q++) before += s_wcnt[q];
    const uint32_t nact = s_wcnt[0] + s_wcnt[1] + s_wcnt[2] + s_wcnt[3];
    if (!nact) {
        if (tid == 0) bsum[blockIdx.x] = 0;
        return;
    }
    if (act) {
        const uint32_t slot = before + (uint32_t)__popcll(am & ((1ull << lane) - 1ull));
        s_slot[slot] = (uint16_t)tid;
        uint32_t hi = 0;
#pragma unroll
        for (int q = 0; q < 4; q++) {
            s_c[slot][q] = r.c[2 * q];
            hi |= (uint32_t)(r.c[2 * q + 1] >> 63) << q;
        }
        s_c[slot][4] = act;
        s_hi[slot] = (uint8_t)hi;
    }
    __syncthreads();
    uint32_t n = 0;
    if ((uint32_t)tid < nact) {
        const uint64_t c0 = s_c[tid][0], c1 = s_c[tid][1], c2 = s_c[tid][2], c3 = s_c[tid][3];
        uint64_t a2 = s_c[tid][4];
        const uint32_t hi = s_hi[tid];
        while (a2) {
            const int b = __builtin_ctzll(a2);
            a2 &= a2 - 1;
            int idx;
            if (b != 63)
                idx = (int)((c0 >> b) & 3ull) | ((int)((c1 >> b) & 3ull) << 2) | ((int)((c2 >> b) & 3ull) << 4) | ((int)((c3 >> b) & 3ull) << 6);
            else
                idx = (int)(c0 >> 63) | ((int)(hi & 1u) << 1) | ((int)(c1 >> 63) << 2) | ((int)(hi >> 1 & 1u) << 3) | ((int)(c2 >> 63) << 4) |
                      ((int)(hi >> 2 & 1u) << 5) | ((int)(c3 >> 63) << 6) | ((int)(hi >> 3 & 1u) << 7);
            n += s_ntri[idx];
        }
        counts[(size_t)blockIdx.x * 256 + s_slot[tid]] = (uint16_t)n;
    }
    uint32_t s = n;
#pragma unroll
    for (int o = 32; o > 0; o >>= 1) s += __shfl_xor(s, o, 64);
    if (lane == 0) s_part[wv] = s;
    __syncthreads();
    if (tid == 0) bsum[blockIdx.x] = s_part[0] + s_part[1] + s_part[2] + s_part[3];
}

__global__ __launch_bounds__(1024) void k_mc_scan(const uint32_t *__restrict__ bsum, size_t n,
                                                  uint64_t *__restrict__ boff, uint32_t *mb, uint32_t seq) {
    __shared__ uint64_t s_wave[16];
    __shared__ uint64_t s_carry;
    __shared__ uint32_t s_tot[64], s_exc[64];
    constexpr int RND = 4;
    const int lane = threadIdx.x & 63, wv = threadIdx.x >> 6;
    const size_t base = (size_t)blockIdx.x * (1024 * 4 * RND);
    uint64_t pre = 0;
    {
        const uint4 *b4 = reinterpret_cast<const uint4 *>(bsum);
        const size_t n4 = base / 4;
        uint64_t p0 = 0, p1 = 0, p2 = 0, p3 = 0;
        size_t i = threadIdx.x;
        for (; i + 3 * 1024 < n4; i += 4 * 1024) {
            const uint4 a = b4[i], b = b4[i + 1024], c = b4[i + 2048], d = b4[i + 3072];
            p0 += (uint64_t)a.x + a.y + a.z + a.w;
            p1 += (uint64_t)b.x + b.y + b.z + b.w;
            p2 += (uint64_t)c.x + c.y + c.z + c.w;
            p3 += (uint64_t)d.x + d.y + d.z + d.w;
        }
        for (; i < n4; i += 1024) {
            const uint4 a = b4[i];
            p0 += (uint64_t)a.x + a.y + a.z + a.w;
        }
        pre = p0 + p1 + p2 + p3;
    }
#pragma unroll
    for (int o = 32; o > 0; o >>= 1) pre += __shfl_xor(pre, o, 64);
    if (lane == 0) s_wave[wv] = pre;
    const bool al16 = ((uintptr_t)bsum & 15) == 0 && ((uintptr_t)boff & 15) == 0;
    uint32_t v[RND][4], inc[RND];
#pragma unroll
    for (int r = 0; r < RND; r++) {
        const size_t i0 = base + (size_t)r * 4096 + (size_t)threadIdx.x * 4;
        if (al16 && i0 + 3 < n) {
            const uint4 a = *reinterpret_cast<const uint4 *>(bsum + i0);
            v[r][0] = a.x; v[r][1] = a.y; v[r][2] = a.z; v[r][3] = a.w;
        } else {
#pragma unroll
            for (int q = 0; q < 4; q++) v[r][q] = i0 + q < n ? bsum[i0 + q] : 0u;
        }
    }
#pragma unroll
    for (int r = 0; r < RND; r++) {
        inc[r] = v[r][0] + v[r][1] + v[r][2] + v[r][3];
#pragma unroll
        for (int o = 1; o < 64; o <<= 1) {
            const uint32_t t = __shfl_up(inc[r], o, 64);
            if (lane >= o) inc[r] += t;
        }
        if (lane == 63) s_tot[r * 16 + wv] = inc[r];
    }
    __syncthreads();
    if (wv == 0) {
        const uint32_t t = s_tot[lane];
        uint32_t e = t;
#pragma unroll
        for (int o = 1; o < 64; o <<= 1) {
            const uint32_t u = __shfl_up(e, o, 64);
            if (lane >= o) e += u;
        }
        s_exc[lane] = e - t;
        uint64_t c = 0;
        for (int q = 0; q < 16; q++) c += s_wave[q];
        if (lane == 0) s_carry = c;
        if (lane == 63 && base + 1024 * 4 * RND >= n) {
            const uint64_t total = c + e;
            boff[n] = total;
            if (mb) {
                mb[0] = (uint32_t)total;
                mb[1] = (uint32_t)(total >> 32);
                __threadfence_system();
                __hip_atomic_store(&mb[63], seq, __ATOMIC_RELEASE, __HIP_MEMORY_SCOPE_SYSTEM);
            }
        }
    }
    __syncthreads();
    const uint64_t carry = s_carry;
#pragma unroll
    for (int r = 0; r < RND; r++) {
// ... 282 lines not shown
}

int mc_inside_planes(const ivx_mc_params *p, const Geom &g, const Scratch &s, const void *a, void *dst, double iso0, double iso1,
                     hipStream_t st) {
    return MC_BY_DTYPE(p->dtype, run_bits, p, g, s, a, (uint8_t *)dst, iso0, iso1, st);
}

int mc_queue_list(const ivx_mc_params *p, const Geom &g, const Scratch &s, const void *scratch_, void *d_list, int64_t max_tris,
                  hipStream_t st) {
    const char *scratch = (const char *)scratch_;
    const uint64_t *boff = (const uint64_t *)(scratch + s.off_boff);
    for (int q = 0; q < p->niso; q++) {
        const uint64_t *bits = mc_bits_ptr(scratch, s, q);
        const uint16_t *counts = (const uint16_t *)(scratch + s.off_counts) + (size_t)q * s.nwords;
        hipLaunchKernelGGL(k_mc_list, dim3((unsigned)s.nblocks), dim3(256), 0, st, bits, g, s.nwords, pad_bits(p, q), counts,
                           boff + (size_t)q * s.nblocks, (uint64_t *)d_list, (uint64_t)max_tris);
        IVX_LAUNCH_CHECK();
    }
    return IVX_OK;
}

int mc_upload_piece(const ivx_mc_params *p, const void *a, const int64_t strides[3], void **d_a, void **d_scr) {
    size_t sb;
    int rc = ivx_dev_mc_scratch_bytes(p, &sb);
    if (rc) return rc;
    const size_t isz = dtype_size(p->dtype);
    const int64_t shape[3] = {p->nz, p->ny, p->nx};
    if ((rc = ws_get(WS_IN, (size_t)p->nz * p->ny * p->nx * isz, d_a))) return rc;
    if ((rc = ws_get(WS_AUX0, sb, d_scr))) return rc;
    return upload_strided(*d_a, a, shape, strides, isz, WS_IN);
}

}

extern "C" int ivx_mc_split_word_ids(const ivx_mc_params *p, const uint32_t *wid, size_t n, uint32_t *k, uint32_t *j, uint32_t *w) {
    Geom g;
    int rc = make_geom(p, &g);
    if (rc) return rc;
    for (size_t i = 0; i < n; i++) mc_split_wid(g, wid[i], k[i], j[i], w[i]);
    return IVX_OK;
}

extern "C" int ivx_dev_mc_scratch_bytes(const ivx_mc_params *p, size_t *nbytes) {
    Geom g;
    int rc = make_geom(p, &g);
    if (rc) return rc;
    *nbytes = make_scratch(g, p->niso).total;
    return IVX_OK;
}

static int mc_read_total(const ivx_mc_params *p, const Scratch &s, void *scratch_, int64_t *ntris, hipStream_t st) {
    char *scratch = (char *)scratch_;
    int rc;
    uint64_t *boff = (uint64_t *)(scratch + s.off_boff);
    const size_t nb = s.nblocks * (size_t)p->niso;
    uint32_t seq, tw[2];
    if (p->niso == 2) {
        uint32_t seq0, t0[2];
        if ((rc = ivx::mailbox_publish(boff + s.nblocks, 2, st, &seq0))) return rc;
        if ((rc = ivx::mailbox_wait(seq0, st, t0, 2))) return rc;
        mc_pieces().set_split(scratch_, ((uint64_t)t0[1] << 32) | t0[0]);
    }
    if ((rc = ivx::mailbox_publish(boff + nb, 2, st, &seq))) return rc;
    if ((rc = ivx::mailbox_wait(seq, st, tw, 2))) return rc;
    *ntris = (int64_t)(((uint64_t)tw[1] << 32) | tw[0]);
    return IVX_OK;
}

static int mc_read_total_early(const ivx_mc_params *p, const Scratch &s, void *scratch_, int64_t *ntris, hipStream_t st) {
    const uint32_t seq = p->niso == 1 ? mc_pieces().total_seq(scratch_) : 0u;
    if (seq) {
        uint32_t tw[2];
        int got = 0;
        const int rc = ivx::mailbox_wait_reserved(seq, st, tw, 2, &got);
        if (rc) return rc;
        if (got) {
            *ntris = (int64_t)(((uint64_t)tw[1] << 32) | tw[0]);
            return IVX_OK;
        }
    }
    return mc_read_total(p, s, scratch_, ntris, st);
}

static int mc_count_impl(const ivx_mc_params *p, const void *a, const uint64_t *inside_bits, void *scratch_, int64_t *ntris,
                         void *stream) {
    Geom g;
    Scratch s;
    bool empty;
    int rc = mc_piece_layout(p, &g, &s, &empty);
    if (rc) return rc;
    IVX_REQUIRE(!inside_bits || p->niso == 1, IVX_EINVAL, "mc_count_bits: one iso-value only");
    if (ntris) *ntris = 0;
    if (empty) return IVX_OK;
    IVX_REQUIRE(a || inside_bits, IVX_EINVAL, "mc_count: neither voxels nor an inside plane");
    char *scratch = (char *)scratch_;
    hipStream_t st = S(stream);
    mc_pieces().begin_count(scratch_, inside_bits);
    if (!inside_bits && (rc = mc_inside_planes(p, g, s, a, scratch + s.off_bits, p->iso[0], p->iso[1], st))) return rc;
    uint32_t *bsum = (uint32_t *)(scratch + s.off_bsum);
    uint64_t *boff = (uint64_t *)(scratch + s.off_boff);
    for (int q = 0; q < p->niso; q++) {
        const uint64_t *bits = mc_bits_ptr(scratch, s, q);
        uint16_t *counts = (uint16_t *)(scratch + s.off_counts) + (size_t)q * s.nwords;
        hipLaunchKernelGGL(k_mc_count, dim3((unsigned)s.nblocks), dim3(256), 0, st, bits, g, s.nwords, pad_bits(p, q),
                           counts, bsum + (size_t)q * s.nblocks);
        IVX_LAUNCH_CHECK();
    }
    const size_t nb = s.nblocks * (size_t)p->niso;
    uint32_t *mb = nullptr, seq = 0;
    if (p->niso == 1) {
        if ((rc = ivx::mailbox_reserve(&mb, &seq))) return rc;
        mc_pieces().set_total_seq(scratch_, seq);
    }
    hipLaunchKernelGGL(k_mc_scan, dim3((unsigned)std::max<size_t>(1, (nb + 16383) / 16384)), dim3(1024), 0, st, bsum, nb, boff, mb,
                       seq);
    IVX_LAUNCH_CHECK();
    return ntris ? mc_read_total_early(p, s, scratch_, ntris, st) : IVX_OK;
}

extern "C" int ivx_dev_mc_count(const ivx_mc_params *p, const void *a, void *scratch_, int64_t *ntris, void *stream) {
    return mc_count_impl(p, a, nullptr, scratch_, ntris, stream);
}
extern "C" int ivx_dev_mc_count_async(const ivx_mc_params *p, const void *a, void *scratch_, void *stream) {
    return mc_count_impl(p, a, nullptr, scratch_, nullptr, stream);
}
extern "C" int ivx_dev_mc_total(const ivx_mc_params *p, void *scratch_, int64_t *ntris, void *stream) {
    Geom g;
    Scratch s;
    bool empty;
    int rc = mc_piece_layout(p, &g, &s, &empty);
    if (rc) return rc;
    *ntris = 0;
    return empty ? IVX_OK : mc_read_total(p, s, scratch_, ntris, S(stream));
}
extern "C" int ivx_dev_mc_total_early(const ivx_mc_params *p, void *scratch_, int64_t *ntris, void *stream) {
    Geom g;
    Scratch s;
    bool empty;
    int rc = mc_piece_layout(p, &g, &s, &empty);
    if (rc) return rc;
    *ntris = 0;
    return empty ? IVX_OK : mc_read_total_early(p, s, scratch_, ntris, S(stream));
}

extern "C" int ivx_dev_mc_count_bits(const ivx_mc_params *p, const uint64_t *inside_bits, void *scratch_, int64_t *ntris,
                                     void *stream) {
    return mc_count_impl(p, nullptr, inside_bits, scratch_, ntris, stream);
}
extern "C" int ivx_dev_mc_count_bits_async(const ivx_mc_params *p, const uint64_t *inside_bits, void *scratch_, void *stream) {
    return mc_count_impl(p, nullptr, inside_bits, scratch_, nullptr, stream);
}

extern "C" int ivx_dev_mc_emit(const ivx_mc_params *p, const void *a, const void *scratch, float *tris,
                               int64_t max_tris, void *stream) {
    Geom g;
    Scratch s;
    bool empty;
    int rc = mc_piece_layout(p, &g, &s, &empty);
    if (rc) return rc;
    if (empty || max_tris <= 0) return IVX_OK;
    return MC_BY_DTYPE(p->dtype, run_emit, p, g, s, a, (const char *)scratch, tris, max_tris, S(stream), nullptr);
}

extern "C" int ivx_dev_mc_emit_levels(const ivx_mc_params *p, const void *scratch, const uint64_t *sel_bits, double v_out,
                                      double v_in, double v_sel, float *tris, int64_t max_tris, void *stream) {
    Geom g;
    Scratch s;
    bool empty;
    int rc = mc_piece_layout(p, &g, &s, &empty);
    if (rc) return rc;
    IVX_REQUIRE(p->dtype == IVX_U8 && p->niso == 1 && sel_bits, IVX_EINVAL, "mc_emit_levels: uint8 mask, one iso-value");
    IVX_REQUIRE(v_out < p->iso[0] && v_in >= p->iso[0] && v_sel >= p->iso[0] && (double)p->pad_value == v_out, IVX_EINVAL,
                "mc_emit_levels: v_out must lie below the iso-value and equal the padding value, v_in and v_sel at or above it");
    if (empty || max_tris <= 0) return IVX_OK;
    const McLevels lv = make_levels(sel_bits, p->iso[0], v_out, v_in, v_sel);
    return run_emit<uint8_t>(p, g, s, nullptr, (const char *)scratch, tris, max_tris, S(stream), &lv);
}

extern "C" int ivx_dev_mc_list(const ivx_mc_params *p, const void *scratch, int64_t max_tris, void *stream) {
    Geom g;
    Scratch s;
    bool empty;
    int rc = mc_piece_layout(p, &g, &s, &empty);
    if (rc) return rc;
    if (empty || max_tris <= 0) return IVX_OK;
    hipStream_t st = S(stream);
    void *d_list;
    if ((rc = ws_get_s(WS_MCLIST, st, (size_t)max_tris * 8 + 64, &d_list))) return rc;
    if ((rc = mc_queue_list(p, g, s, scratch, d_list, max_tris, st))) return rc;
    mc_pieces().list_built(scratch, d_list, max_tris);
    return IVX_OK;
}

extern "C" int ivx_marching_cubes(const ivx_mc_params *p, const void *a, const int64_t strides[3], float *tris,
                                  int64_t max_tris, int64_t *ntris) {
    HostCallGuard host_guard__;
    void *d_a, *d_scr;
    int rc = mc_upload_piece(p, a, strides, &d_a, &d_scr);
    if (rc) return rc;
    int64_t cnt = 0;
// ... 46 lines not shown
```

invesalius3_amd/device.py:

```python
from __future__ import annotations

import ctypes
import os
from typing import NamedTuple, Optional

import numpy as np

from . import _lib as L


class _MaskLevels(NamedTuple):
    v_in: float
    sel: Optional[ctypes.c_void_p]
    v_sel: float

    @property
    def has_second(self):
        return self.sel is not None


class DeviceBuffer:

    def __init__(self, nbytes: int):
        self.nbytes = int(nbytes)
        p = ctypes.c_void_p()
        L.check(L.lib().ivx_malloc(ctypes.byref(p), ctypes.c_size_t(max(self.nbytes, 16))), "ivx_malloc")
        self.ptr = p

    def upload(self, a: np.ndarray):
        a = np.ascontiguousarray(a)
        assert a.nbytes <= self.nbytes
        L.check(L.lib().ivx_memcpy_h2d(self.ptr, L.ptr(a), ctypes.c_size_t(a.nbytes)))

    def upload_view(self, a: np.ndarray):
        a = np.asarray(a)
        if a.ndim > 3 or a.itemsize not in (1, 2, 4, 8) or a.ndim == 0:
            return self.upload(a)
        assert a.nbytes <= self.nbytes
        pad = 3 - a.ndim
        L.check(L.lib().ivx_upload_strided(self.ptr, L.ptr(a), L.i64((1,) * pad + a.shape),
                                           L.i64((a.strides[0] * a.shape[0],) * pad + a.strides), a.itemsize), "upload_view")

    def download_view(self, out: np.ndarray):
        if out.ndim > 3 or out.itemsize not in (1, 2, 4, 8) or out.ndim == 0:
            out[...] = self.download(out.shape, out.dtype)
            return out
        assert out.nbytes <= self.nbytes
        pad = 3 - out.ndim
        L.check(L.lib().ivx_download_strided(L.ptr(out), L.i64((1,) * pad + out.shape),
                                             L.i64((out.strides[0] * out.shape[0],) * pad + out.strides), self.ptr, out.itemsize),
                "download_view")
        return out

    def download(self, shape, dtype, out: np.ndarray | None = None) -> np.ndarray:
        if out is None:
            out = np.empty(shape, dtype)
        else:
            n = int(np.prod(shape)) * np.dtype(dtype).itemsize
            assert out.flags["C_CONTIGUOUS"] and out.nbytes >= n
            out = out.reshape(-1).view(np.uint8)[:n].view(dtype).reshape(shape)
        assert out.nbytes <= self.nbytes
        L.check(L.lib().ivx_memcpy_d2h(L.ptr(out), self.ptr, ctypes.c_size_t(out.nbytes)))
        return out

    def zero(self, stream=None, nbytes=None):
        L.check(L.lib().ivx_memset(self.ptr, 0, ctypes.c_size_t(self.nbytes if nbytes is None else nbytes), stream))

    def at(self, offset_bytes: int) -> ctypes.c_void_p:
        return ctypes.c_void_p(self.ptr.value + int(offset_bytes))

    def close(self):
        if self.ptr is not None and self.ptr.value:
            L.lib().ivx_free(self.ptr)
        self.ptr = None

    def __del__(self):
        try:
            self.close()
        except Exception:
            pass


class TrackedBuffer(DeviceBuffer):

    def __init__(self, nbytes: int, on_touch, on_read=None):
        self._on_touch = self._on_read = None
        super().__init__(nbytes)
        self._on_touch, self._on_read = on_touch, on_read

    @property
    def ptr(self):
# ... 40 lines not shown

        def __exit__(self, *a):
            return False

    _OFF = _Off()

    def _ev(self):
        if self._pool:
            return self._pool.pop()
        e = ctypes.c_void_p()
        L.check(L.lib().ivx_event_create(ctypes.byref(e)))
        return e

    class _Span:
        def __init__(self, t, name):
            self.t, self.name = t, name

        def __enter__(self):
            self.e0 = self.t._ev()
            L.check(L.lib().ivx_event_record(self.e0, self.t.stream))

        def __exit__(self, *a):
            e1 = self.t._ev()
            L.check(L.lib().ivx_event_record(e1, self.t.stream))
            self.t.spans.append((self.name, self.e0, e1))

    def records(self, name) -> bool:
        return self.only is None or name in self.only

    def span(self, name):
        if not self.records(name):
            return Timer._OFF
        return Timer._Span(self, name)

    def collect(self) -> dict:
        out = {}
        for name, e0, e1 in self.spans:
            ms = ctypes.c_float(0)
            L.check(L.lib().ivx_event_elapsed_ms(e0, e1, ctypes.byref(ms)))
            out.setdefault(name, []).append(ms.value)
            self._pool += [e0, e1]
        self.spans = []
        return out


class DeviceVolume:

    def __init__(self, image: np.ndarray | None = None, shape=None, spacing=(1.0, 1.0, 1.0), device: int | None = None):
        L.require_device()
        if device is not None:
            L.set_device(device)
        if image is not None:
            if image.dtype != np.int16 or image.ndim != 3:
                raise TypeError("image must be a 3-D int16 array")
            shape = image.shape
        self.shape = tuple(int(s) for s in shape)
        self.dz, self.dy, self.dx = self.shape
        self.n = self.dz * self.dy * self.dx
        self.spacing = tuple(float(s) for s in spacing)
        s = ctypes.c_void_p()
        L.check(L.lib().ivx_stream_create(ctypes.byref(s)))
        self.stream = s
        self.timer = Timer(self.stream)
        self._mbits_valid = False
        self._mbits_range = None
        self._mask_levels = None
        self._out_bytes_zero = False
        self._mc_params_cache = {}
        self._stream2 = None
        self._sync_events = []
        self._prefetch = None
        self._gate = None
        self._gate_epoch = 0
        self._gate_armed = False
        self._mbits_version = 0
        self._out_pending = None
        self._mask_pending = False
        self._defer_pays = True
        self._fuse = os.environ.get("IVX_NO_FUSE", "") == ""
        self._apply_levels = os.environ.get("IVX_APPLY_LEVELS", "1") != "0"
        self._use_ranges = os.environ.get("IVX_RANGES", "1") != "0"
        self._mask_defer = os.environ.get("IVX_MASK_DEFER", "1") != "0"
        self._select = os.environ.get("IVX_FLOOD_SELECT", "1") != "0"
        self._look_ahead = -1
        self._ranges = None
        self._ranges_valid = False
        self.image = TrackedBuffer(self.n * 2, self._image_touched)
        self.mask = TrackedBuffer(self.n, self._mask_touched, self._mask_read)
        self.out_mask = TrackedBuffer(self.n, self._out_touched)
        if image is not None:
            self.image.upload_view(image)
        self.mask.zero(self.stream)
        self.zero_out_mask()
        self.plan = L.FloodPlan(self.dz, self.dy, self.dx, (self.dx + 63) // 64, 0)
        nb, ns = ctypes.c_size_t(0), ctypes.c_size_t(0)
        L.check(L.lib().ivx_flood_bits_bytes(ctypes.byref(self.plan), ctypes.byref(nb)))
        L.check(L.lib().ivx_flood_scratch_bytes(ctypes.byref(self.plan), ctypes.byref(ns)))
        self.cand = DeviceBuffer(nb.value)
        self.reached = DeviceBuffer(nb.value)
        self._mbits = DeviceBuffer(nb.value)
        self._plane_words = nb.value // 8
        self.flood_scratch = DeviceBuffer(ns.value)
        self._mc_scratch = None
        self._tris = None
        self._verts = None
        self._faces = None
        self._range_buf = None
        self._range_valid = False
        self.sync()

    def _image_touched(self):
        self._mbits_range = None
        self._range_valid = False
        self._ranges_valid = False
        self._drop_volren()

    def _mask_touched(self):
        self._mask_read()
        self._mp_cells_valid = False
        self._mbits_valid = False
        self._mbits_range = None
        self._mask_levels = None
        self._mbits_version += 1

    def _materialize_mask(self):
        if self._mask_pending:
            self._defer_pays = False
            lv = self._mask_levels
            sel = self.reached.ptr if lv[1] is not None else None
            with self.timer.span("mask_bytes"):
                L.check(L.lib().ivx_dev_mask_from_planes(ctypes.byref(self.plan), self._mbits.ptr, sel, self.mask.raw, int(lv[0]),
                                                         int(lv[0] if lv[1] is None else lv[1]), self.stream), "mask_from_planes")
            self._mask_pending = False

    def _mask_read(self):
        if self._mask_pending:
            self._materialize_mask()
            self.sync()

    def mask_bytes(self) -> ctypes.c_void_p:
        self._materialize_mask()
        return self.mask.raw

    def _out_logically_zero(self) -> bool:
        return self._out_bytes_zero and self._out_pending is None

    def _materialize_out(self):
        if self._out_pending is not None:
            L.check(L.lib().ivx_dev_flood_apply(ctypes.byref(self.plan), self.reached.ptr, L.U8, self.out_mask.raw,
                                                ctypes.c_double(self._out_pending), self.stream))
            self._out_pending = None
            self._out_bytes_zero = False

    def _out_touched(self):
        self._materialize_out()
        self._out_bytes_zero = False

    def zero_out_mask(self):
        self._materialize_mask()
        if not self._out_bytes_zero:
            L.check(L.lib().ivx_memset(self.out_mask.raw, 0, ctypes.c_size_t(self.n), self.stream))
        self._out_bytes_zero, self._out_pending = True, None

    def sync(self):
        self._materialize_mask()
        L.check(L.lib().ivx_stream_synchronize(self.stream))
# ... 49 lines not shown
        from . import history

        return history.snapshot_device(self.mask_bytes(), self.n, self.shape, self.stream)

    def restore_mask(self, snapshot):
        if snapshot.closed:
            raise ValueError("restore_mask: the snapshot has been closed")
        if snapshot.n != self.n or tuple(snapshot.shape) != self.shape:
            raise ValueError("restore_mask: the snapshot holds shape %r, the volume has %r" % (tuple(snapshot.shape), self.shape))
        self._materialize_mask()
        L.check(L.lib().ivx_dev_mask_snapshot_restore(self.mask.raw, self.n, snapshot.header.ptr, snapshot.pool.ptr,
                                                      snapshot.literal_blocks, 1, None, self.stream), "restore_mask")
        self._mask_touched()

    def download_out_mask(self) -> np.ndarray:
        self._materialize_mask()
        self._materialize_out()
        self.sync()
        return self.out_mask.download(self.shape, np.uint8)

    def threshold(self, lo: int, hi: int, preserve: bool = False):
        lib = L.lib()
        self._join_prefetch()
        if self._fuse and not preserve and self.dx % 64 == 0:
            self._mbits_version += 1
            self._mp_cells_valid = False
            dims = (c64(self.dz), c64(self.dy), c64(self.dx), int(lo), int(hi))
            defer = self._mask_defer and self._defer_pays
            if self._use_ranges:
                mode = 1 if self._ranges_valid else 0
                if defer:
                    L.check(lib.ivx_dev_threshold_i16_plane_ranges(self.image.raw, *dims, self._mbits.ptr, self._ranges_buffer().ptr,
                                                                   mode, self.stream), "threshold")
                else:
                    L.check(lib.ivx_dev_threshold_i16_bits_ranges(self.image.raw, *dims, self.mask.raw, self._mbits.ptr,
                                                                  self._ranges_buffer().ptr, mode, self.stream), "threshold")
                self._ranges_valid = True
            elif defer:
                L.check(lib.ivx_dev_threshold_i16_plane(self.image.raw, *dims, self._mbits.ptr, self.stream), "threshold")
            else:
                L.check(lib.ivx_dev_threshold_i16_bits(self.image.raw, *dims, self.mask.raw, self._mbits.ptr, self.stream), "threshold")
            self._mask_pending = defer
            self._mbits_valid, self._mbits_range = True, (int(lo), int(hi))
            self._mask_levels = (255, None)
            return
        if preserve:
            self._materialize_mask()
        self._mask_pending = False
        L.check(lib.ivx_dev_threshold_i16(self.image.raw, c64(self.dz), c64(self.dy), c64(self.dx), int(lo), int(hi),
                                          int(bool(preserve)), None, self.mask.raw, self.stream), "threshold")
        self._mask_touched()

    def _ranges_buffer(self) -> DeviceBuffer:
        if self._ranges is None:
            nb = ctypes.c_size_t(0)
            L.check(L.lib().ivx_image_ranges_bytes(c64(self.dz), c64(self.dy), c64(self.dx), ctypes.byref(nb)), "image_ranges_bytes")
            self._ranges = DeviceBuffer(max(nb.value, 4))
            self._ranges_valid = False
        return self._ranges

    def lut_image_255(self, ww, wl) -> DeviceBuffer:
        self._materialize_mask()
        buf = DeviceBuffer(self.n * 2)
        L.check(L.lib().ivx_dev_lut_i16(self.image.raw, c64(self.n), ctypes.c_double(float(ww)), ctypes.c_double(float(wl)),
                                        1, buf.ptr, self.stream), "lut_image_255")
        return buf

    def region_grow(self, seeds_xyz, t0, t1, strct, fill: int = 1, select_value: int | None = 254,
                    image: DeviceBuffer | None = None) -> int:
        lib = L.lib()
        img_ptr = image.ptr if image is not None else self.image.raw
        s3 = np.ascontiguousarray(strct, dtype=np.uint8)
        bits = ctypes.c_uint32(0)
        L.check(lib.ivx_flood_strct_bits(L.ptr(s3), L.i64(s3.shape), ctypes.byref(bits)))
        self.plan.strct_bits = bits.value
        seeds = np.ascontiguousarray(np.array([tuple(s) for s in seeds_xyz], dtype=np.int64).reshape(-1, 3))
        p = ctypes.byref(self.plan)
        st = self.stream
        t0, t1 = float(int(t0)), float(int(t1))
        self._before_flood()
        cand, shared = self._candidate_plane(image, t0, t1, fill)
        rounds = ctypes.c_int(0)
        write = self._flood_write(fill, select_value) if self._select else None
        if write is not None:
            L.check(lib.ivx_dev_flood_grow_select(p, L.I16, img_ptr, ctypes.c_double(t0), ctypes.c_double(t1), L.ptr(seeds),
                                                  c64(len(seeds)), cand.ptr, self.reached.ptr, self.flood_scratch.ptr,
                                                  ctypes.byref(rounds), ctypes.byref(write), int(self._look_ahead), st), "region_grow")
        else:
            L.check(lib.ivx_dev_flood_grow(p, L.I16, img_ptr, ctypes.c_double(t0), ctypes.c_double(t1), L.ptr(seeds),
                                           c64(len(seeds)), cand.ptr, self.reached.ptr, self.flood_scratch.ptr,
                                           ctypes.byref(rounds), st), "region_grow")
        self._gate_armed = False
        self._apply_reached(fill, select_value, shared, queued=write is not None)
        return rounds.value

    def flood_visits(self):
        self._materialize_mask()
        return L.flood_visits(self.plan, self.flood_scratch.ptr, self.stream)

    def _before_flood(self):
        self._materialize_out()
        if self._mask_levels is not None and self._mask_levels[1] is not None:
            self._materialize_mask()
            self._mask_levels = None

    def _candidate_plane(self, image, t0, t1, fill):
        shared = (image is None and self._mbits_valid and self._out_logically_zero() and int(fill) != 0
                  and self._mbits_range == (int(t0), int(t1)))
        if shared:
            return self._mbits, True
        bar, bar_mode = (None, 0) if (self._out_logically_zero() and (int(fill) & 0xff) != 0) else (self.out_mask.raw, 1)
        if image is None and self._use_ranges and self._ranges_valid:
            L.check(L.lib().ivx_dev_flood_candidates_ranges(ctypes.byref(self.plan), self.image.raw, ctypes.c_double(t0),
                                                            ctypes.c_double(t1), bar, bar_mode, ctypes.c_double(fill),
                                                            self._ranges.ptr, self.cand.ptr, self.stream), "flood_candidates_ranges")
            return self.cand, False
        img_ptr = image.ptr if image is not None else self.image.raw
        L.check(L.lib().ivx_dev_flood_candidates(ctypes.byref(self.plan), L.I16, img_ptr, ctypes.c_double(t0),
                                                 ctypes.c_double(t1), bar, bar_mode, ctypes.c_double(fill),
                                                 self.cand.ptr, self.stream))
        return self.cand, False

    def _write_kind(self, fill, select_value):
        if not (self._out_logically_zero() and int(fill) != 0):
            return None
        if select_value is not None and self._mask_levels == (255, None) and self._mbits_valid and self._apply_levels:
            return L.FLOOD_WRITE_MASK_FROM_PLANES if self._mask_pending else L.FLOOD_WRITE_APPLY_LEVELS
        return L.FLOOD_WRITE_APPLY_U8 if select_value is not None else L.FLOOD_WRITE_NONE

    def _flood_write(self, fill, select_value):
        kind = self._write_kind(fill, select_value)
        if kind is None or (kind == L.FLOOD_WRITE_MASK_FROM_PLANES and self.timer.records("mask_bytes")):
            return None
        if kind == L.FLOOD_WRITE_APPLY_U8:
            self._materialize_mask()
        return L.FloodWrite(kind=kind, v_in=255, v_sel=int(select_value) if select_value is not None else 0,
                            inside_bits=self._mbits.ptr.value, mask=self.mask.raw.value)

    def _apply_reached(self, fill, select_value, shared, queued=False):
        lib, p, st = L.lib(), ctypes.byref(self.plan), self.stream
        if select_value is not None:
            self._mp_cells_valid = False
        kind = self._write_kind(fill, select_value)
        assert kind is not None or not queued
        if kind not in (L.FLOOD_WRITE_MASK_FROM_PLANES, L.FLOOD_WRITE_APPLY_LEVELS):
            self._materialize_mask()
        else:
            self._defer_pays = True
        if kind is not None:
            self._out_pending = int(fill)
            if kind == L.FLOOD_WRITE_MASK_FROM_PLANES:
                if not queued:
                    with self.timer.span("mask_bytes"):
                        L.check(lib.ivx_dev_mask_from_planes(p, self._mbits.ptr, self.reached.ptr, self.mask.raw, 255,
                                                             int(select_value), st), "mask_from_planes")
                self._mask_pending = False
            elif kind == L.FLOOD_WRITE_APPLY_LEVELS and not queued:
                L.check(lib.ivx_dev_flood_apply_levels(p, self.reached.ptr, self._mbits.ptr, self.mask.raw, 255, int(select_value), st),
                        "flood_apply_levels")
            elif kind == L.FLOOD_WRITE_APPLY_U8 and not queued:
                L.check(lib.ivx_dev_flood_apply(p, self.reached.ptr, L.U8, self.mask.raw, ctypes.c_double(int(select_value)), st))
        elif select_value is not None:
            L.check(lib.ivx_dev_flood_apply2(p, self.reached.ptr, self.out_mask.raw, int(fill), self.mask.raw,
                                             int(select_value), st))
            self._out_bytes_zero = False
        else:
            L.check(lib.ivx_dev_flood_apply(p, self.reached.ptr, L.U8, self.out_mask.raw, ctypes.c_double(fill), st))
            self._out_bytes_zero = False
        if select_value is not None:
            lv = self._mask_levels
            self._mask_levels = (lv[0], int(select_value)) if (lv is not None and lv[1] is None and int(select_value) >= 127
                                                                and self._mbits_valid) else None
        if select_value is not None and self._mbits_valid and not (shared and int(select_value) >= 127):
            self._join_prefetch()
            self._mbits_version += 1
            L.check(lib.ivx_dev_bits_combine(self._mbits.ptr, self.reached.ptr, c64(self._plane_words),
                                             0 if int(select_value) >= 127 else 1, st))
# ... 257 lines not shown

    def swap_axes(self, axes):
        from .slice_ import swapped_spacing

        a, b = (int(v) for v in axes)
        if a == b or not {a, b} <= {0, 1, 2}:
            raise ValueError("axes must be two different ones of 0, 1, 2")
        self._join_prefetch()
        out = DeviceBuffer(self.n * 2)
        try:
            L.check(L.lib().ivx_dev_image_swap_axes(self.image.raw, c64(self.dz), c64(self.dy), c64(self.dx), 2, a, b, out.ptr, self.stream),
                    "swap_axes")
            L.check(L.lib().ivx_memcpy_d2d(self.image.raw, out.ptr, ctypes.c_size_t(self.n * 2), self.stream), "swap_axes copy")
            L.check(L.lib().ivx_stream_synchronize(self.stream))
        finally:
            out.close()
        shape = list(self.shape)
        shape[a], shape[b] = shape[b], shape[a]
        self._after_image_geometry(shape, swapped_spacing(self.spacing, (a, b)))

    def fix_gantry_tilt(self, tilt, scratch_bytes: int | None = None):
        from .slice_ import gantry_tilt_shifts

        shifts = gantry_tilt_shifts(self.dz, self.spacing, tilt)
        cvals = np.zeros(self.dz, np.int32)
        if self.n == 0:
            return cvals
        nb = ctypes.c_size_t(0)
        L.check(L.lib().ivx_image_tilt_scratch_bytes(c64(self.dz), c64(self.dy), c64(self.dx), ctypes.byref(nb)), "tilt_scratch_bytes")
        self._join_prefetch()
        scratch = DeviceBuffer(nb.value if scratch_bytes is None else int(scratch_bytes))
        try:
            L.check(L.lib().ivx_dev_image_fix_gantry_tilt(self.image.raw, c64(self.dz), c64(self.dy), c64(self.dx), L.ptr(shifts),
                                                          scratch.ptr, ctypes.c_size_t(scratch.nbytes), L.ptr(cvals), self.stream),
                    "fix_gantry_tilt")
            L.check(L.lib().ivx_stream_synchronize(self.stream))
        finally:
            scratch.close()
        self._after_image_geometry()
        return cvals

    def reached_count(self) -> int:
        self._materialize_mask()
        n = ctypes.c_int64(0)
        L.check(L.lib().ivx_dev_flood_count(ctypes.byref(self.plan), self.reached.ptr, ctypes.byref(n), self.stream))
        return n.value

    def _mc_params(self, from_binary, min_value, max_value, fill_border_holes=True, z0=0, z1=None, roi_start=None,
                   pad_bottom=None, pad_top=None) -> L.McParams:
        z1 = self.dz if z1 is None else z1
        key = (bool(from_binary), min_value, max_value, bool(fill_border_holes), z0, z1, roi_start, pad_bottom, pad_top,
               tuple(self.spacing))
        hit = self._mc_params_cache.get(key)
        if hit is not None:
            return hit
        p = L.McParams()
        pb = (z0 == 0) if pad_bottom is None else pad_bottom
        pt = (z1 >= self.dz) if pad_top is None else pad_top
        if fill_border_holes:
            p.pad_xy, p.pad_bottom, p.pad_top, p.vtk_pz = 1, int(pb), int(pt), int(pb)
        else:
            p.pad_xy = p.pad_bottom = p.pad_top = p.vtk_pz = 0
        p.nz, p.ny, p.nx = z1 - z0, self.dy, self.dx
        p.roi_start = z0 if roi_start is None else roi_start
        p.spacing[:] = self.spacing
        if from_binary:
            p.dtype, p.niso, p.pad_value = L.U8, 1, 0.0
            p.iso[:] = [127.0, 0.0]
        else:
            p.dtype, p.niso, p.pad_value = L.I16, 2, float(np.iinfo(np.int16).min)
            p.iso[:] = [float(min_value), float(max_value)]
        if len(self._mc_params_cache) < 64:
            self._mc_params_cache[key] = p
        return p

    def _surface_params(self, from_binary, min_value, max_value, fill_border_holes):
        return self._mc_params(from_binary, min_value, max_value, fill_border_holes), 0

    def _mc_setup(self, p, z0):
        nb = ctypes.c_size_t(0)
        L.check(L.lib().ivx_dev_mc_scratch_bytes(ctypes.byref(p), ctypes.byref(nb)))
        if self._mc_scratch is None or self._mc_scratch.nbytes < nb.value:
            self._join_prefetch()
            if self._mc_scratch is not None:
                self.sync()
                self._mc_scratch.close()
            self._mc_scratch = DeviceBuffer(nb.value)
        isz = 1 if p.dtype == L.U8 else 2
        src = (self.mask if p.dtype == L.U8 else self.image).raw_at(z0 * self.dy * self.dx * isz)
        plane = None
        if (p.dtype == L.U8 and p.niso == 1 and p.iso[0] == 127.0 and self._mbits_valid and p.ny == self.dy
                and p.nx == self.dx):
            plane = self._mbits.at(z0 * self.dy * ((self.dx + 63) // 64) * 8)
        return src, plane

    def _levels(self, p, plane, z0):
        lv = self._mask_levels
        if not (plane is not None and lv is not None and self._fuse and os.environ.get("IVX_MC_LEVELS", "1") != "0"
                and float(p.pad_value) == 0.0 and lv[0] > 127 and (lv[1] is None or lv[1] > 127)):
            return None
        if lv[1] is None:
            return _MaskLevels(float(lv[0]), None, float(lv[0]))
        return _MaskLevels(float(lv[0]), self.reached.at(z0 * self.dy * ((self.dx + 63) // 64) * 8), float(lv[1]))

    def _emit(self, p, src, plane, z0, cap, stream):
        lib, levels = L.lib(), self._levels(p, plane, z0)
        if levels is not None:
            sel = levels.sel if levels.has_second else plane
            L.check(lib.ivx_dev_mc_emit_levels(ctypes.byref(p), self._mc_scratch.ptr, sel, ctypes.c_double(0.0),
                                               ctypes.c_double(levels.v_in), ctypes.c_double(levels.v_sel), self._tris.ptr, c64(cap),
                                               stream), "mc_emit")
        else:
            L.check(lib.ivx_dev_mc_emit(ctypes.byref(p), src, self._mc_scratch.ptr, self._tris.ptr, c64(cap), stream), "mc_emit")

    def _second_stream(self):
        if self._stream2 is None:
            s = ctypes.c_void_p()
            if os.environ.get("IVX_PREFETCH_PRIORITY", "low") == "low":
                L.check(L.lib().ivx_stream_create_low_priority(ctypes.byref(s)))
            else:
                L.check(L.lib().ivx_stream_create(ctypes.byref(s)))
            self._stream2 = s
            for _ in range(2):
                e = ctypes.c_void_p()
                L.check(L.lib().ivx_event_create_sync(ctypes.byref(e)))
                self._sync_events.append(e)
        return self._stream2

    def _join_prefetch(self):
        if self._prefetch is not None:
            if self._gate_armed:
                L.check(L.lib().ivx_dev_gate_open(self._gate.ptr, ctypes.c_uint32(self._gate_epoch), self.stream))
                L.check(L.lib().ivx_dev_flood_disarm_gate(self.flood_scratch.ptr))
                self._gate_armed = False
            L.check(L.lib().ivx_stream_synchronize(self._stream2))
            self._prefetch = None

    def surface_prefetch(self, from_binary=True, min_value=0, max_value=0, fill_border_holes=True,
                         behind_flood: bool = True) -> bool:
        if not from_binary or not self._fuse or self._tris is None or not self._mbits_valid:
            return False
        self._join_prefetch()
        p, z0 = self._surface_params(from_binary, min_value, max_value, fill_border_holes)
        src, plane = self._mc_setup(p, z0)
        if plane is None:
            return False
        lib, s2 = L.lib(), self._second_stream()
        cap = self._tris.nbytes // 36
        L.check(lib.ivx_event_record(self._sync_events[0], self.stream))
        L.check(lib.ivx_stream_wait_event(s2, self._sync_events[0]))
        if behind_flood:
            if self._gate is None:
                self._gate = DeviceBuffer(64)
                self._gate.zero(self.stream)
                self.sync()
            self._gate_epoch = (self._gate_epoch % 0x7fffffff) + 1
            L.check(lib.ivx_dev_flood_arm_gate(self.flood_scratch.ptr, self._gate.ptr, ctypes.c_uint32(self._gate_epoch),
                                               ctypes.c_uint32(512)))
            L.check(lib.ivx_dev_gate_wait(self._gate.ptr, ctypes.c_uint32(self._gate_epoch), ctypes.c_uint32(300), s2))
            self._gate_armed = True
        L.check(lib.ivx_dev_mc_count_bits_async(ctypes.byref(p), plane, self._mc_scratch.ptr, s2), "mc_count")
        L.check(lib.ivx_dev_mc_list(ctypes.byref(p), self._mc_scratch.ptr, c64(cap), s2), "mc_list")
        self._prefetch = (p, z0, cap, self._mbits_version)
        return True

    def marching_cubes(self, from_binary=True, min_value=0, max_value=0, fill_border_holes=True, download=False,
                       params: L.McParams | None = None, z0: int = 0, out: np.ndarray | None = None):
        self._materialize_mask()
        lib = L.lib()
        if params is not None:
            p = params
        else:
            p, z0 = self._surface_params(from_binary, min_value, max_value, fill_border_holes)
        pf, n = self._prefetch, ctypes.c_int64(0)
        if pf is not None:
            ok = (pf[0] is p and pf[1] == z0 and self._tris is not None and pf[2] == self._tris.nbytes // 36
                  and pf[3] == self._mbits_version and self._mbits_valid)
            if not ok:
                self._join_prefetch()
            else:
                src, plane = self._mc_setup(p, z0)
                s2, cap = self._stream2, pf[2]
                if self._gate_armed:
                    L.check(lib.ivx_dev_gate_open(self._gate.ptr, ctypes.c_uint32(self._gate_epoch), self.stream))
                    L.check(lib.ivx_dev_flood_disarm_gate(self.flood_scratch.ptr))
                    self._gate_armed = False
                L.check(lib.ivx_event_record(self._sync_events[1], self.stream))
                L.check(lib.ivx_stream_wait_event(s2, self._sync_events[1]))
                L.check(lib.ivx_dev_mc_emit(ctypes.byref(p), src, self._mc_scratch.ptr, self._tris.ptr, c64(cap), s2), "mc_emit")
                L.check(lib.ivx_dev_mc_total(ctypes.byref(p), self._mc_scratch.ptr, ctypes.byref(n), s2), "mc_total")
                self._prefetch = None
                nt = n.value
                if nt <= cap:
                    if download:
                        return self._tris.download((nt, 3, 3), np.float32, out if out is not None and out.nbytes >= nt * 36 else None)
                    return nt
        src, plane = self._mc_setup(p, z0)
        n = ctypes.c_int64(0)
        if self._tris is not None:
            cap = self._tris.nbytes // 36
            with self.timer.span("mc_count"):
                if plane is not None:
                    L.check(lib.ivx_dev_mc_count_bits_async(ctypes.byref(p), plane, self._mc_scratch.ptr, self.stream), "mc_count")
                else:
                    L.check(lib.ivx_dev_mc_count_async(ctypes.byref(p), src, self._mc_scratch.ptr, self.stream), "mc_count")
            with self.timer.span("mc_emit"):
                self._emit(p, src, plane, z0, cap, self.stream)
            L.check(lib.ivx_dev_mc_total_early(ctypes.byref(p), self._mc_scratch.ptr, ctypes.byref(n), self.stream), "mc_total")
            nt = n.value
            if nt > cap:
                self.sync()
                self._tris.close()
                self._tris = DeviceBuffer(int(nt * 36 * 1.25) + 4096)
                self._emit(p, src, plane, z0, nt, self.stream)
        else:
            with self.timer.span("mc_count"):
                if plane is not None:
                    L.check(lib.ivx_dev_mc_count_bits(ctypes.byref(p), plane, self._mc_scratch.ptr, ctypes.byref(n), self.stream),
                            "mc_count")
                else:
                    L.check(lib.ivx_dev_mc_count(ctypes.byref(p), src, self._mc_scratch.ptr, ctypes.byref(n), self.stream), "mc_count")
            nt = n.value
            self._tris = DeviceBuffer(int(nt * 36 * 1.25) + 4096)
            with self.timer.span("mc_emit"):
                self._emit(p, src, plane, z0, nt, self.stream)
        if download:
            self.sync()
            return self._tris.download((nt, 3, 3), np.float32, out if out is not None and out.nbytes >= nt * 36 else None)
        return nt

    def marching_cubes_indexed(self, from_binary=True, min_value=0, max_value=0, fill_border_holes=True, download=False,
                               params: L.McParams | None = None, z0: int = 0):
        self._materialize_mask()
        lib = L.lib()
        if params is not None:
            p = params
        else:
            p, z0 = self._surface_params(from_binary, min_value, max_value, fill_border_holes)
        self._join_prefetch()
        src, plane = self._mc_setup(p, z0)
        nt, nv = ctypes.c_int64(0), ctypes.c_int64(0)
        with self.timer.span("mc_count"):
            if plane is not None:
                L.check(lib.ivx_dev_mc_count_bits(ctypes.byref(p), plane, self._mc_scratch.ptr, ctypes.byref(nt), self.stream),
                        "mc_count")
            else:
                L.check(lib.ivx_dev_mc_count(ctypes.byref(p), src, self._mc_scratch.ptr, ctypes.byref(nt), self.stream), "mc_count")
        levels = self._levels(p, plane, z0)
        with self.timer.span("mci_count"):
            if levels is not None:
                L.check(lib.ivx_dev_mc_indexed_count_levels(ctypes.byref(p), self._mc_scratch.ptr, ctypes.byref(nv), self.stream),
                        "mc_indexed_count")
            else:
                L.check(lib.ivx_dev_mc_indexed_count(ctypes.byref(p), src, self._mc_scratch.ptr, ctypes.byref(nv), self.stream),
                        "mc_indexed_count")
        for name, need in (("_verts", nv.value * 12), ("_faces", nt.value * 12)):
            buf = getattr(self, name)
            if buf is None or buf.nbytes < need:
                if buf is not None:
                    buf.close()
                setattr(self, name, DeviceBuffer(int(need * 1.25) + 4096))
        with self.timer.span("mci_emit"):
            if levels is not None:
                L.check(lib.ivx_dev_mc_indexed_emit_levels(ctypes.byref(p), self._mc_scratch.ptr, levels.sel, ctypes.c_double(0.0),
                                                           ctypes.c_double(levels.v_in), ctypes.c_double(levels.v_sel), self._verts.ptr,
                                                           c64(nv.value), self._faces.ptr, c64(nt.value), self.stream),
                        "mc_indexed_emit")
            else:
                L.check(lib.ivx_dev_mc_indexed_emit(ctypes.byref(p), src, self._mc_scratch.ptr, self._verts.ptr, c64(nv.value),
                                                    self._faces.ptr, c64(nt.value), self.stream), "mc_indexed_emit")
        if download:
            self.sync()
            return self._verts.download((nv.value, 3), np.float32), self._faces.download((nt.value, 3), np.int32)
        return nv.value, nt.value

    def watershed(self, markers: np.ndarray, strct, use_ww_wl: bool = False, wl=0, ww=0, overwrite: bool = False,
                  algorithm: str = "Watershed IFT", mg_size=(3, 3, 3)):
        self._materialize_mask()
        mk = np.ascontiguousarray(markers)
        if mk.shape != self.shape or mk.dtype.type not in (np.int8, np.int16):
            raise TypeError("markers must be an int8 / int16 array of the volume's shape")
        s3 = np.zeros((3, 3, 3), np.uint8)
        s3[:] = np.asarray(strct).astype(bool)
        lib, n = L.lib(), self.n
        d_mk, d_cost, d_lab = DeviceBuffer(mk.nbytes), DeviceBuffer(n * 2), DeviceBuffer(n)
        d_mk.upload(mk)
        try:
            if use_ww_wl:
                L.check(lib.ivx_dev_lut_u16(self.image.raw, c64(n), ctypes.c_double(float(ww)), ctypes.c_double(float(wl)), 0,
                                            d_cost.ptr, self.stream), "lut")
            else:
                mm = DeviceBuffer(64)
                L.check(lib.ivx_dev_minmax_f32(L.I16, self.image.raw, c64(n), mm.ptr, self.stream))
                self.sync()
                imin = int(mm.download((2,), np.float32)[0])
                mm.close()
                L.check(lib.ivx_dev_shift_min_u16(self.image.raw, c64(n), imin, d_cost.ptr, self.stream), "min shift")
            stats = (ctypes.c_int64 * 16)()
            mdt = L.I16 if mk.dtype == np.int16 else L.I8
            if algorithm == "Watershed":
                d_grad = DeviceBuffer(n * 2)
                try:
                    gsz = (ctypes.c_int * 3)(*[int(v) for v in mg_size])
                    L.check(lib.ivx_dev_morph_gradient_u16(d_cost.ptr, c64(self.dz), c64(self.dy), c64(self.dx), gsz, d_grad.ptr,
                                                           self.stream), "gradient")
                    with self.timer.span("watershed_flood"):
                        L.check(lib.ivx_dev_watershed_sk(d_grad.ptr, mdt, d_mk.ptr, c64(self.dz), c64(self.dy), c64(self.dx), L.ptr(s3),
                                                         None, None, d_lab.ptr, None, stats, self.stream), "watershed_sk")
                    self.sync()
                finally:
                    d_grad.close()
            else:
                with self.timer.span("watershed_flood"):
                    L.check(lib.ivx_dev_watershed_ift(d_cost.ptr, mdt, d_mk.ptr, c64(self.dz), c64(self.dy), c64(self.dx), L.ptr(s3),
                                                      None, d_lab.ptr, None, stats, self.stream), "watershed_ift")
            L.check(lib.ivx_dev_watershed_merge(self.mask.ptr, d_lab.ptr, c64(n), int(bool(overwrite)), self.stream), "merge")
            self.sync()
        finally:
            for b in (d_mk, d_cost, d_lab):
                b.close()
        names = (("rounds", "tile_visits", "levels", "generations", "markers", "generation0", "tied_markers_of_different_labels")
                 if algorithm == "Watershed" else ("rounds", "tile_visits", "levels", "time_stamps", "markers", "entries", "tiles"))
# ... 277 lines not shown
```

Baseline: 430,300 Mvoxel/s.

## Fuse mask-levels write into marching-cubes count kernel after region grow

When a region grow ends with a levels mask write and the next surface call will reuse the same MC parameters, the levels write is carried inside the MC count kernel. That kernel counts triangles from the inside bits while storing the mask bytes. The later marching-cubes call then skips its separate count launch, saving one kernel launch and a pass over the bit planes. In exchange it adds Python bookkeeping (RideBook) that arms, takes and drops the fused count against params identity and mask version. Correctness now depends on those invalidation paths catching every case.

```diff
diff --git a/include/ivx.h b/include/ivx.h
--- a/include/ivx.h
+++ b/include/ivx.h
@@ -413,6 +413,10 @@
 int ivx_dev_flood_grow_select(const ivx_flood_plan *p, int dtype, const void *data, double t0, double t1,
                               const int64_t *seeds_xyz, int64_t nseeds, uint64_t *cand, uint64_t *reached, void *scratch,
                               int *rounds, const ivx_flood_write *write, int look_ahead, void *stream);
+int ivx_dev_flood_grow_select_count(const ivx_flood_plan *p, int dtype, const void *data, double t0, double t1,
+                                    const int64_t *seeds_xyz, int64_t nseeds, uint64_t *cand, uint64_t *reached, void *scratch,
+                                    int *rounds, const ivx_flood_write *write, int look_ahead, const ivx_mc_params *mc,
+                                    void *mc_scratch, int *counted, void *stream);
 int ivx_flood_look_ahead(int64_t n_list, int32_t *look_ahead);
 int ivx_dev_flood_apply2(const ivx_flood_plan *p, const uint64_t *reached, uint8_t *out, int fill, uint8_t *mask,
                          int select, void *stream);
diff --git a/invesalius3_amd/_lib.py b/invesalius3_amd/_lib.py
--- a/invesalius3_amd/_lib.py
+++ b/invesalius3_amd/_lib.py
@@ -88,6 +88,10 @@
                        ("ivx_dev_flood_grow_select", [ctypes.POINTER(FloodPlan), ctypes.c_int, c_vp, ctypes.c_double, ctypes.c_double,
                                                       c_vp, c_i64, c_vp, c_vp, c_vp, ctypes.POINTER(ctypes.c_int),
                                                       ctypes.POINTER(FloodWrite), ctypes.c_int, c_vp]),
+                       ("ivx_dev_flood_grow_select_count", [ctypes.POINTER(FloodPlan), ctypes.c_int, c_vp, ctypes.c_double, ctypes.c_double,
+                                                            c_vp, c_i64, c_vp, c_vp, c_vp, ctypes.POINTER(ctypes.c_int),
+                                                            ctypes.POINTER(FloodWrite), ctypes.c_int, ctypes.POINTER(McParams), c_vp,
+                                                            ctypes.POINTER(ctypes.c_int), c_vp]),
                        ("ivx_flood_look_ahead", [c_i64, ctypes.POINTER(ctypes.c_int32)]),
                        ("ivx_dev_image_flip", [c_vp, c_i64, c_i64, c_i64, sz, ctypes.c_int, c_vp]),
                        ("ivx_image_flip", [c_vp, i64p, i64p, sz, ctypes.c_int]),
diff --git a/invesalius3_amd/csrc/ivx_internal.h b/invesalius3_amd/csrc/ivx_internal.h
--- a/invesalius3_amd/csrc/ivx_internal.h
+++ b/invesalius3_amd/csrc/ivx_internal.h
@@ -92,6 +92,13 @@
 int flood_run(const ivx_flood_plan *p, const uint64_t *planes, FloodMode mode, uint64_t *reached, void *scratch, int *rounds,
               void *stream);
 
+struct ApplyWhen;
+bool mc_ride_ok(const ivx_mc_params *p, const void *scratch, int64_t dz, int64_t dy, int64_t dx);
+void mc_ride_begin(void *scratch, const uint64_t *inside_bits);
+int mc_ride_launch(const ivx_mc_params *p, void *scratch, const uint64_t *reached, const uint64_t *inside, int64_t nchunks, uint8_t *mask,
+                   int v_in, int v_sel, bool all, const ApplyWhen &when, hipStream_t st);
+int mc_ride_scan(const ivx_mc_params *p, void *scratch, hipStream_t st);
+
 int mailbox_publish(const void *dsrc, int ndwords, hipStream_t st, uint32_t *seq_out);
 int mailbox_wait(uint32_t seq, hipStream_t st, uint32_t *out, int ndwords);
 int mailbox_reserve(uint32_t **slot_out, uint32_t *seq_out);
diff --git a/invesalius3_amd/csrc/k_flood.hip b/invesalius3_amd/csrc/k_flood.hip
--- a/invesalius3_amd/csrc/k_flood.hip
+++ b/invesalius3_amd/csrc/k_flood.hip
@@ -4,7 +4,10 @@
 #include <stdlib.h>
 
 #include "flood_tiles.h"
+#include "levels_write.h"
 #include "words_from_records.h"
+
+using ivx::ApplyWhen;
 
 namespace {
 
@@ -984,40 +987,17 @@
     }
 }
 
-struct ApplyWhen {
-    const unsigned int *next_len;
-    unsigned long long *line;
-    unsigned long long report;
-};
 template <bool ALL>
 __global__ __launch_bounds__(256) void k_flood_apply_levels16(const uint16_t *__restrict__ reached, const uint16_t *__restrict__ inside,
                                                               int64_t nchunks, uint4 *__restrict__ out, uint8_t v_in, uint8_t v_sel,
                                                               ApplyWhen when) {
-    if (when.next_len) {
-        if (*when.next_len != 0u) return;
-        if (blockIdx.x == 0 && threadIdx.x == 0) __hip_atomic_store(&when.line[2], when.report, __ATOMIC_RELAXED, __HIP_MEMORY_SCOPE_SYSTEM);
-    }
+    if (ivx::apply_when_skips(when)) return;
     const int64_t stride = (int64_t)gridDim.x * 1024;
     const unsigned int in4 = 0x01010101u * v_in, sel4 = 0x01010101u * v_sel;
     for (int64_t i0 = (int64_t)blockIdx.x * 1024 + threadIdx.x; i0 < nchunks; i0 += stride) {
-        unsigned int m[4], b[4];
-#pragma unroll
-        for (int u = 0; u < 4; u++) {
-            const int64_t i = i0 + u * 256;
-            m[u] = i < nchunks && (!ALL || reached) ? reached[i] : 0u;
-            b[u] = i < nchunks ? inside[i] : 0u;
-        }
-#pragma unroll
-        for (int u = 0; u < 4; u++) {
-            if (ALL ? i0 + u * 256 >= nchunks : !m[u]) continue;
-            auto bytes = [](unsigned int bits4) { return ((bits4 * 0x00204081u) & 0x01010101u) * 0xffu; };
-            auto word = [&](unsigned int r4, unsigned int i4) {
-                const unsigned int rs = bytes(r4);
-                return (sel4 & rs) | (in4 & bytes(i4) & ~rs);
-            };
-            out[i0 + u * 256] = make_uint4(word(m[u] & 15u, b[u] & 15u), word(m[u] >> 4 & 15u, b[u] >> 4 & 15u),
-                                           word(m[u] >> 8 & 15u, b[u] >> 8 & 15u), word(m[u] >> 12 & 15u, b[u] >> 12 & 15u));
-        }
+        ivx::LevelsWords w;
+        ivx::levels_load<ALL>(reached, inside, nchunks, i0, w);
+        ivx::levels_store<ALL>(w, nchunks, i0, out, in4, sel4);
     }
 }
 
@@ -1367,10 +1347,15 @@
     }
     return IVX_OK;
 }
+struct McRide {
+    const ivx_mc_params *p;
+    void *scratch;
+};
 static int launch_levels(const Tiles &t, const uint64_t *reached, const uint64_t *inside, uint8_t *mask, int v_in, int v_sel, bool all,
-                         const ApplyWhen &when, hipStream_t st) {
+                         const ApplyWhen &when, hipStream_t st, const McRide *ride = nullptr) {
     const int64_t nchunks = t.dz * t.dy * t.dx / 16;
     if (!nchunks) return IVX_OK;
+    if (ride) return ivx::mc_ride_launch(ride->p, ride->scratch, reached, inside, nchunks, mask, v_in, v_sel, all, when, st);
     const int64_t blocks = ivx::cdiv(nchunks, 1024);
     auto k = all ? k_flood_apply_levels16<true> : k_flood_apply_levels16<false>;
     hipLaunchKernelGGL(k, dim3((unsigned)(blocks < 16384 ? blocks : 16384)), dim3(256), 0, st, (const uint16_t *)reached,
@@ -1383,6 +1368,8 @@
 struct EarlyWrite {
     const ivx_flood_write *w;
     bool written;
+    const McRide *ride = nullptr;
+    bool plain = false;
 };
 constexpr unsigned EARLY_BELOW = 96u;
 constexpr int EARLY_TRIES = 2;
@@ -1419,6 +1406,7 @@
     if (sym && flood_mode_ccl() && ivx::ccl_supported(p->strct_bits)) {
         if (rounds) *rounds = 1;
         IVX_HIP(hipMemsetAsync(dirty[0], 0, (size_t)t.ntiles, st));
+        if (early) early->plain = true;
         return ivx::ccl_run(p, cand, reached, scratch_, st);
     }
     int total_rounds = 0;
@@ -1517,7 +1505,7 @@
             early_report = ((unsigned long long)tag << 56) | ((unsigned long long)(queued & 0xffffff) << 32) | 1ull;
             if (trace) fprintf(stderr, "ivx flood: write queued behind round %lld\n", (long long)queued);
             rc = launch_levels(t, reached, early->w->inside_bits, early->w->mask, early->w->v_in, early->w->v_sel, early_all,
-                               ApplyWhen{cnt + queued % RING, (unsigned long long *)line, early_report}, st);
+                               ApplyWhen{cnt + queued % RING, (unsigned long long *)line, early_report}, st, early->ride);
             if (rc) return rc;
         }
         prev_list = n_list;
@@ -1527,6 +1515,7 @@
             IVX_HIP(hipMemsetAsync(dirty[1], 0, (size_t)t.ntiles, st));
             if ((rc = ivx::ccl_run(p, cand, reached, scratch_, st))) return rc;
             total_rounds += 1;
+            if (early) early->plain = true;
             break;
         }
         IVX_REQUIRE(total_rounds < (1 << 24) - 64, IVX_EHIP, "flood: did not converge");
@@ -1771,23 +1760,64 @@
     return launch_levels(t, reached, inside_bits, mask, v_in, v_sel, true, ApplyWhen{nullptr, nullptr, 0ull}, ivx::S(stream));
 }
 
+static int grow_select_impl(const ivx_flood_plan *p, int dtype, const void *data, double t0, double t1, const int64_t *seeds_xyz,
+                            int64_t nseeds, uint64_t *cand, uint64_t *reached, void *scratch_, int *rounds, const ivx_flood_write *write,
+                            int look_ahead, const ivx_mc_params *mc, void *mc_scratch, int *counted, void *stream) {
+    IVX_REQUIRE(write && write->kind >= IVX_FLOOD_WRITE_NONE && write->kind <= IVX_FLOOD_WRITE_APPLY_U8, IVX_EINVAL,
+                "flood_grow_select: no write description, or one of an unknown kind");
+    IVX_REQUIRE(write->kind == IVX_FLOOD_WRITE_NONE || write->mask, IVX_EINVAL, "flood_grow_select: the write has no mask");
+    if (counted) *counted = 0;
+    EarlyWrite early = {write, false};
+    const bool all = write->kind == IVX_FLOOD_WRITE_MASK_FROM_PLANES;
+    const McRide ride = {mc, mc_scratch};
+    Tiles t;
+    int rc = make_tiles(p, &t);
+    if (rc) return rc;
+    if (mc && counted && (all || write->kind == IVX_FLOOD_WRITE_APPLY_LEVELS) &&
+        levels_check(t, reached, write->inside_bits, write->mask, write->v_in, write->v_sel, all) == IVX_OK &&
+        ivx::mc_ride_ok(mc, mc_scratch, t.dz, t.dy, t.dx)) {
+        early.ride = &ride;
+        ivx::mc_ride_begin(mc_scratch, write->inside_bits);
+    }
+    rc = flood_grow_impl(p, dtype, data, t0, t1, seeds_xyz, nseeds, cand, reached, scratch_, rounds, stream, look_ahead, &early);
+    if (rc) return rc;
+    const bool fused = early.ride && !early.plain;
+    if (!early.written) {
+        switch (write->kind) {
+        case IVX_FLOOD_WRITE_MASK_FROM_PLANES:
+        case IVX_FLOOD_WRITE_APPLY_LEVELS:
+            if (fused)
+                rc = launch_levels(t, reached, write->inside_bits, write->mask, write->v_in, write->v_sel, all, ApplyWhen{nullptr, nullptr, 0ull},
+                                   ivx::S(stream), &ride);
+            else if (all)
+                rc = ivx_dev_mask_from_planes(p, write->inside_bits, reached, write->mask, write->v_in, write->v_sel, stream);
+            else
+                rc = ivx_dev_flood_apply_levels(p, reached, write->inside_bits, write->mask, write->v_in, write->v_sel, stream);
+            break;
+        case IVX_FLOOD_WRITE_APPLY_U8: rc = ivx_dev_flood_apply(p, reached, IVX_U8, write->mask, (double)write->v_sel, stream); break;
+        default: break;
+        }
+        if (rc) return rc;
+    }
+    if (fused) {
+        if ((rc = ivx::mc_ride_scan(mc, mc_scratch, ivx::S(stream)))) return rc;
+        *counted = 1;
+    }
+    return IVX_OK;
+}
 extern "C" int ivx_dev_flood_grow_select(const ivx_flood_plan *p, int dtype, const void *data, double t0, double t1,
                                          const int64_t *seeds_xyz, int64_t nseeds, uint64_t *cand, uint64_t *reached,
                                          void *scratch_, int *rounds, const ivx_flood_write *write, int look_ahead, void *stream) {
-    IVX_REQUIRE(write && write->kind >= IVX_FLOOD_WRITE_NONE && write->kind <= IVX_FLOOD_WRITE_APPLY_U8, IVX_EINVAL,
-                "flood_grow_select: no write description, or one of an unknown kind");
-    IVX_REQUIRE(write->kind == IVX_FLOOD_WRITE_NONE || write->mask, IVX_EINVAL, "flood_grow_select: the write has no mask");
-    EarlyWrite early = {write, false};
-    int rc = flood_grow_impl(p, dtype, data, t0, t1, seeds_xyz, nseeds, cand, reached, scratch_, rounds, stream, look_ahead, &early);
-    if (rc || early.written) return rc;
-    switch (write->kind) {
-    case IVX_FLOOD_WRITE_MASK_FROM_PLANES:
-        return ivx_dev_mask_from_planes(p, write->inside_bits, reached, write->mask, write->v_in, write->v_sel, stream);
-    case IVX_FLOOD_WRITE_APPLY_LEVELS:
-        return ivx_dev_flood_apply_levels(p, reached, write->inside_bits, write->mask, write->v_in, write->v_sel, stream);
-    case IVX_FLOOD_WRITE_APPLY_U8: return ivx_dev_flood_apply(p, reached, IVX_U8, write->mask, (double)write->v_sel, stream);
-    default: return IVX_OK;
-    }
+    return grow_select_impl(p, dtype, data, t0, t1, seeds_xyz, nseeds, cand, reached, scratch_, rounds, write, look_ahead, nullptr, nullptr,
+                            nullptr, stream);
+}
+extern "C" int ivx_dev_flood_grow_select_count(const ivx_flood_plan *p, int dtype, const void *data, double t0, double t1,
+                                               const int64_t *seeds_xyz, int64_t nseeds, uint64_t *cand, uint64_t *reached,
+                                               void *scratch_, int *rounds, const ivx_flood_write *write, int look_ahead,
+                                               const ivx_mc_params *mc, void *mc_scratch, int *counted, void *stream) {
+    IVX_REQUIRE(mc && mc_scratch && counted, IVX_EINVAL, "flood_grow_select_count: null piece, scratch or result");
+    return grow_select_impl(p, dtype, data, t0, t1, seeds_xyz, nseeds, cand, reached, scratch_, rounds, write, look_ahead, mc, mc_scratch,
+                            counted, stream);
 }
 
 extern "C" int ivx_dev_flood_apply2(const ivx_flood_plan *p, const uint64_t *reached, uint8_t *out, int fill,
diff --git a/invesalius3_amd/csrc/k_mc.hip b/invesalius3_amd/csrc/k_mc.hip
--- a/invesalius3_amd/csrc/k_mc.hip
+++ b/invesalius3_amd/csrc/k_mc.hip
@@ -1,5 +1,6 @@
 #include <algorithm>
 
+#include "levels_write.h"
 #include "mc_common.h"
 
 #define MC_TABLE_QUAL static __device__ __attribute__((aligned(16))) const
@@ -198,9 +199,15 @@
     return r;
 }
 
-__global__ __launch_bounds__(256) void k_mc_count(const uint64_t *__restrict__ bits, Geom g, size_t nwords,
-                                                  uint64_t pbits, uint16_t *__restrict__ counts,
-                                                  uint32_t *__restrict__ bsum) {
+struct McRideArgs {
+    const uint16_t *reached, *inside;
+    int64_t nchunks;
+    uint4 *out;
+    unsigned int in4, sel4;
+};
+template <bool RIDE, bool ALL>
+__device__ __forceinline__ void mc_count_body(const uint64_t *__restrict__ bits, const Geom &g, size_t nwords, uint64_t pbits,
+                                              uint16_t *__restrict__ counts, uint32_t *__restrict__ bsum, const McRideArgs &ride) {
     __shared__ uint32_t s_part[4], s_wcnt[4];
     __shared__ uint8_t s_ntri[256];
     __shared__ uint64_t s_c[256][5];
@@ -208,6 +215,23 @@
     __shared__ uint16_t s_slot[256];
     const int tid = threadIdx.x, lane = tid & 63, wv = tid >> 6;
     const uint8_t ntri = MC_NTRI[tid];
+    const int64_t ride_i0 = (int64_t)blockIdx.x * 1024 + tid;
+    LevelsWords lw;
+    if (RIDE) levels_load<ALL>(ride.reached, ride.inside, ride.nchunks, ride_i0, lw);
+    auto ride_rest = [&]() {
+        if (!RIDE) return;
+        const int64_t stride = (int64_t)gridDim.x * 1024;
+        for (int64_t i0 = ride_i0 + stride; i0 < ride.nchunks; i0 += stride) {
+            LevelsWords w2;
+            levels_load<ALL>(ride.reached, ride.inside, ride.nchunks, i0, w2);
+            levels_store<ALL>(w2, ride.nchunks, i0, ride.out, ride.in4, ride.sel4);
+        }
+    };
+    auto ride_store = [&]() {
+#if !defined(IVX_RIDE_NO_STORES)
+        if (RIDE) levels_store<ALL>(lw, ride.nchunks, ride_i0, ride.out, ride.in4, ride.sel4);
+#endif
+    };
     const size_t wid = (size_t)blockIdx.x * 256 + tid;
     uint64_t act = 0;
     Corner8 r;
@@ -218,6 +242,9 @@
         act = r.active;
         if (!act) counts[wid] = 0;
     }
+#if defined(IVX_RIDE_STORES_EARLY)
+    ride_store();
+#endif
     const unsigned long long am = __ballot(act != 0);
     if (lane == 0) s_wcnt[wv] = (uint32_t)__popcll(am);
     s_ntri[tid] = ntri;
@@ -225,8 +252,19 @@
     uint32_t before = 0;
     for (int q = 0; q < wv; q++) before += s_wcnt[q];
     const uint32_t nact = s_wcnt[0] + s_wcnt[1] + s_wcnt[2] + s_wcnt[3];
+#if !defined(IVX_RIDE_STORES_EARLY)
+    ride_store();
+#endif
+#if defined(IVX_RIDE_NO_WALK)
+    if (RIDE) {
+        if (tid == 0) bsum[blockIdx.x] = 0;
+        ride_rest();
+        return;
+    }
+#endif
     if (!nact) {
         if (tid == 0) bsum[blockIdx.x] = 0;
+        ride_rest();
         return;
     }
     if (act) {
@@ -266,6 +304,19 @@
     if (lane == 0) s_part[wv] = s;
     __syncthreads();
     if (tid == 0) bsum[blockIdx.x] = s_part[0] + s_part[1] + s_part[2] + s_part[3];
+    ride_rest();
+}
+__global__ __launch_bounds__(256) void k_mc_count(const uint64_t *__restrict__ bits, Geom g, size_t nwords,
+                                                  uint64_t pbits, uint16_t *__restrict__ counts,
+                                                  uint32_t *__restrict__ bsum) {
+    mc_count_body<false, false>(bits, g, nwords, pbits, counts, bsum, McRideArgs{});
+}
+template <bool ALL>
+__global__ __launch_bounds__(256) void k_mc_count_write(const uint64_t *__restrict__ bits, Geom g, size_t nwords, uint64_t pbits,
+                                                        uint16_t *__restrict__ counts, uint32_t *__restrict__ bsum, McRideArgs ride,
+                                                        ApplyWhen when) {
+    if (apply_when_skips(when)) return;
+    mc_count_body<true, ALL>(bits, g, nwords, pbits, counts, bsum, ride);
 }
 
 __global__ __launch_bounds__(1024) void k_mc_scan(const uint32_t *__restrict__ bsum, size_t n,
@@ -714,6 +765,36 @@
     return mc_read_total(p, s, scratch_, ntris, st);
 }
 
+static void mc_count_record(void *scratch_, const uint64_t *inside_bits) { mc_pieces().begin_count(scratch_, inside_bits); }
+static int mc_count_launch(const ivx_mc_params *p, const Geom &g, const Scratch &s, void *scratch_, hipStream_t st) {
+    char *scratch = (char *)scratch_;
+    uint32_t *bsum = (uint32_t *)(scratch + s.off_bsum);
+    for (int q = 0; q < p->niso; q++) {
+        const uint64_t *bits = mc_bits_ptr(scratch, s, q);
+        uint16_t *counts = (uint16_t *)(scratch + s.off_counts) + (size_t)q * s.nwords;
+        hipLaunchKernelGGL(k_mc_count, dim3((unsigned)s.nblocks), dim3(256), 0, st, bits, g, s.nwords, pad_bits(p, q),
+                           counts, bsum + (size_t)q * s.nblocks);
+        IVX_LAUNCH_CHECK();
+    }
+    return IVX_OK;
+}
+static int mc_count_scan(const ivx_mc_params *p, const Scratch &s, void *scratch_, hipStream_t st) {
+    char *scratch = (char *)scratch_;
+    uint32_t *bsum = (uint32_t *)(scratch + s.off_bsum);
+    uint64_t *boff = (uint64_t *)(scratch + s.off_boff);
+    const size_t nb = s.nblocks * (size_t)p->niso;
+    uint32_t *mb = nullptr, seq = 0;
+    if (p->niso == 1) {
+        int rc = ivx::mailbox_reserve(&mb, &seq);
+        if (rc) return rc;
+        mc_pieces().set_total_seq(scratch_, seq);
+    }
+    hipLaunchKernelGGL(k_mc_scan, dim3((unsigned)std::max<size_t>(1, (nb + 16383) / 16384)), dim3(1024), 0, st, bsum, nb, boff, mb,
+                       seq);
+    IVX_LAUNCH_CHECK();
+    return IVX_OK;
+}
+
 static int mc_count_impl(const ivx_mc_params *p, const void *a, const uint64_t *inside_bits, void *scratch_, int64_t *ntris,
                          void *stream) {
     Geom g;
@@ -727,27 +808,45 @@
     IVX_REQUIRE(a || inside_bits, IVX_EINVAL, "mc_count: neither voxels nor an inside plane");
     char *scratch = (char *)scratch_;
     hipStream_t st = S(stream);
-    mc_pieces().begin_count(scratch_, inside_bits);
+    mc_count_record(scratch_, inside_bits);
     if (!inside_bits && (rc = mc_inside_planes(p, g, s, a, scratch + s.off_bits, p->iso[0], p->iso[1], st))) return rc;
-    uint32_t *bsum = (uint32_t *)(scratch + s.off_bsum);
-    uint64_t *boff = (uint64_t *)(scratch + s.off_boff);
-    for (int q = 0; q < p->niso; q++) {
-        const uint64_t *bits = mc_bits_ptr(scratch, s, q);
-        uint16_t *counts = (uint16_t *)(scratch + s.off_counts) + (size_t)q * s.nwords;
-        hipLaunchKernelGGL(k_mc_count, dim3((unsigned)s.nblocks), dim3(256), 0, st, bits, g, s.nwords, pad_bits(p, q),
-                           counts, bsum + (size_t)q * s.nblocks);
-        IVX_LAUNCH_CHECK();
-    }
-    const size_t nb = s.nblocks * (size_t)p->niso;
-    uint32_t *mb = nullptr, seq = 0;
-    if (p->niso == 1) {
-        if ((rc = ivx::mailbox_reserve(&mb, &seq))) return rc;
-        mc_pieces().set_total_seq(scratch_, seq);
-    }
-    hipLaunchKernelGGL(k_mc_scan, dim3((unsigned)std::max<size_t>(1, (nb + 16383) / 16384)), dim3(1024), 0, st, bsum, nb, boff, mb,
-                       seq);
+    if ((rc = mc_count_launch(p, g, s, scratch_, st))) return rc;
+    if ((rc = mc_count_scan(p, s, scratch_, st))) return rc;
+    return ntris ? mc_read_total_early(p, s, scratch_, ntris, st) : IVX_OK;
+}
+
+bool ivx::mc_ride_ok(const ivx_mc_params *p, const void *scratch, int64_t dz, int64_t dy, int64_t dx) {
+    Geom g;
+    Scratch s;
+    bool empty;
+    if (!p || !scratch || mc_piece_layout(p, &g, &s, &empty) != IVX_OK || empty) return false;
+    return p->niso == 1 && p->ny == dy && p->nx == dx && p->nz <= dz;
+}
+void ivx::mc_ride_begin(void *scratch, const uint64_t *inside_bits) { mc_count_record(scratch, inside_bits); }
+int ivx::mc_ride_launch(const ivx_mc_params *p, void *scratch_, const uint64_t *reached, const uint64_t *inside, int64_t nchunks,
+                        uint8_t *mask, int v_in, int v_sel, bool all, const ApplyWhen &when, hipStream_t st) {
+    Geom g;
+    Scratch s;
+    bool empty;
+    int rc = mc_piece_layout(p, &g, &s, &empty);
+    if (rc) return rc;
+    IVX_REQUIRE(!empty && p->niso == 1 && nchunks > 0, IVX_EINVAL, "mc_ride: an empty piece or volume, or two iso-values");
+    char *scratch = (char *)scratch_;
+    const McRideArgs ride = {(const uint16_t *)reached, (const uint16_t *)inside, nchunks, (uint4 *)mask, 0x01010101u * (uint8_t)v_in,
+                             0x01010101u * (uint8_t)v_sel};
+    auto k = all ? k_mc_count_write<true> : k_mc_count_write<false>;
+    hipLaunchKernelGGL(k, dim3((unsigned)s.nblocks), dim3(256), 0, st, mc_bits_ptr(scratch, s, 0), g, s.nwords, pad_bits(p, 0),
+                       (uint16_t *)(scratch + s.off_counts), (uint32_t *)(scratch + s.off_bsum), ride, when);
     IVX_LAUNCH_CHECK();
-    return ntris ? mc_read_total_early(p, s, scratch_, ntris, st) : IVX_OK;
+    return IVX_OK;
+}
+int ivx::mc_ride_scan(const ivx_mc_params *p, void *scratch, hipStream_t st) {
+    Geom g;
+    Scratch s;
+    bool empty;
+    int rc = mc_piece_layout(p, &g, &s, &empty);
+    if (rc) return rc;
+    return mc_count_scan(p, s, scratch, st);
 }
 
 extern "C" int ivx_dev_mc_count(const ivx_mc_params *p, const void *a, void *scratch_, int64_t *ntris, void *stream) {
diff --git a/invesalius3_amd/csrc/levels_write.h b/invesalius3_amd/csrc/levels_write.h
--- /dev/null
+++ b/invesalius3_amd/csrc/levels_write.h
@@ -0,0 +1,51 @@
+#pragma once
+#include <hip/hip_runtime.h>
+#include <stdint.h>
+
+namespace ivx {
+
+struct ApplyWhen {
+    const unsigned int *next_len;
+    unsigned long long *line;
+    unsigned long long report;
+};
+__device__ __forceinline__ bool apply_when_skips(const ApplyWhen &when) {
+    if (when.next_len) {
+        if (*when.next_len != 0u) return true;
+        if (blockIdx.x == 0 && threadIdx.x == 0) __hip_atomic_store(&when.line[2], when.report, __ATOMIC_RELAXED, __HIP_MEMORY_SCOPE_SYSTEM);
+    }
+    return false;
+}
+
+struct LevelsWords {
+    unsigned int m[4], b[4];
+};
+
+template <bool ALL>
+__device__ __forceinline__ void levels_load(const uint16_t *__restrict__ reached, const uint16_t *__restrict__ inside, int64_t nchunks,
+                                            int64_t i0, LevelsWords &w) {
+#pragma unroll
+    for (int u = 0; u < 4; u++) {
+        const int64_t i = i0 + u * 256;
+        w.m[u] = i < nchunks && (!ALL || reached) ? reached[i] : 0u;
+        w.b[u] = i < nchunks ? inside[i] : 0u;
+    }
+}
+
+template <bool ALL>
+__device__ __forceinline__ void levels_store(const LevelsWords &w, int64_t nchunks, int64_t i0, uint4 *__restrict__ out, unsigned int in4,
+                                             unsigned int sel4) {
+#pragma unroll
+    for (int u = 0; u < 4; u++) {
+        if (ALL ? i0 + u * 256 >= nchunks : !w.m[u]) continue;
+        auto bytes = [](unsigned int bits4) { return ((bits4 * 0x00204081u) & 0x01010101u) * 0xffu; };
+        auto word = [&](unsigned int r4, unsigned int i4) {
+            const unsigned int rs = bytes(r4);
+            return (sel4 & rs) | (in4 & bytes(i4) & ~rs);
+        };
+        out[i0 + u * 256] = make_uint4(word(w.m[u] & 15u, w.b[u] & 15u), word(w.m[u] >> 4 & 15u, w.b[u] >> 4 & 15u),
+                                       word(w.m[u] >> 8 & 15u, w.b[u] >> 8 & 15u), word(w.m[u] >> 12 & 15u, w.b[u] >> 12 & 15u));
+    }
+}
+
+}
diff --git a/invesalius3_amd/device.py b/invesalius3_amd/device.py
--- a/invesalius3_amd/device.py
+++ b/invesalius3_amd/device.py
@@ -7,6 +7,7 @@
 import numpy as np
 
 from . import _lib as L
+from .mc_ride import RideBook
 
 
 class _MaskLevels(NamedTuple):
@@ -213,6 +214,7 @@
         self._use_ranges = os.environ.get("IVX_RANGES", "1") != "0"
         self._mask_defer = os.environ.get("IVX_MASK_DEFER", "1") != "0"
         self._select = os.environ.get("IVX_FLOOD_SELECT", "1") != "0"
+        self._ride = RideBook(os.environ.get("IVX_MC_RIDE", "1") != "0")
         self._look_ahead = -1
         self._ranges = None
         self._ranges_valid = False
@@ -428,7 +430,19 @@
         cand, shared = self._candidate_plane(image, t0, t1, fill)
         rounds = ctypes.c_int(0)
         write = self._flood_write(fill, select_value) if self._select else None
-        if write is not None:
+        piece = self._piece_to_ride(write, shared, select_value)
+        if piece is not None:
+            counted = ctypes.c_int(0)
+            L.check(lib.ivx_dev_flood_grow_select_count(p, L.I16, img_ptr, ctypes.c_double(t0), ctypes.c_double(t1), L.ptr(seeds),
+                                                        c64(len(seeds)), cand.ptr, self.reached.ptr, self.flood_scratch.ptr,
+                                                        ctypes.byref(rounds), ctypes.byref(write), int(self._look_ahead),
+                                                        ctypes.byref(piece[0]), self._mc_scratch.ptr, ctypes.byref(counted), st),
+                    "region_grow")
+            if counted.value:
+                self._ride.rode(self._mbits_version)
+            else:
+                self._ride.drop()
+        elif write is not None:
             L.check(lib.ivx_dev_flood_grow_select(p, L.I16, img_ptr, ctypes.c_double(t0), ctypes.c_double(t1), L.ptr(seeds),
                                                   c64(len(seeds)), cand.ptr, self.reached.ptr, self.flood_scratch.ptr,
                                                   ctypes.byref(rounds), ctypes.byref(write), int(self._look_ahead), st), "region_grow")
@@ -439,6 +453,17 @@
         self._gate_armed = False
         self._apply_reached(fill, select_value, shared, queued=write is not None)
         return rounds.value
+
+    def _piece_to_ride(self, write, shared, select_value):
+        if (write is None or write.kind not in (L.FLOOD_WRITE_MASK_FROM_PLANES, L.FLOOD_WRITE_APPLY_LEVELS) or not shared
+                or select_value is None or int(select_value) < 127 or not self._fuse or self._prefetch is not None
+                or self._mc_scratch is None or self._tris is None or self.timer.records("mc_count")
+                or self.timer.records("mask_bytes")):
+            return None
+        piece = self._ride.piece_to_ride()
+        if piece is None or piece[1] != 0 or piece[0].ny != self.dy or piece[0].nx != self.dx or piece[0].nz > self.dz:
+            return None
+        return piece
 
     def flood_visits(self):
         self._materialize_mask()
@@ -862,6 +887,7 @@
         L.check(L.lib().ivx_dev_mc_scratch_bytes(ctypes.byref(p), ctypes.byref(nb)))
         if self._mc_scratch is None or self._mc_scratch.nbytes < nb.value:
             self._join_prefetch()
+            self._ride.drop()
             if self._mc_scratch is not None:
                 self.sync()
                 self._mc_scratch.close()
@@ -925,6 +951,7 @@
         src, plane = self._mc_setup(p, z0)
         if plane is None:
             return False
+        self._ride.drop()
         lib, s2 = L.lib(), self._second_stream()
         cap = self._tris.nbytes // 36
         L.check(lib.ivx_event_record(self._sync_events[0], self.stream))
@@ -977,13 +1004,20 @@
                     return nt
         src, plane = self._mc_setup(p, z0)
         n = ctypes.c_int64(0)
+        if plane is not None and self._tris is not None and not self.timer.records("mc_count"):
+            rode = self._ride.take(p, z0, self._mbits_version)
+        else:
+            rode = False
+            self._ride.drop()
+        self._ride.surface_counted(p, z0, plane is not None)
         if self._tris is not None:
             cap = self._tris.nbytes // 36
-            with self.timer.span("mc_count"):
-                if plane is not None:
-                    L.check(lib.ivx_dev_mc_count_bits_async(ctypes.byref(p), plane, self._mc_scratch.ptr, self.stream), "mc_count")
-                else:
-                    L.check(lib.ivx_dev_mc_count_async(ctypes.byref(p), src, self._mc_scratch.ptr, self.stream), "mc_count")
+            if not rode:
+                with self.timer.span("mc_count"):
+                    if plane is not None:
+                        L.check(lib.ivx_dev_mc_count_bits_async(ctypes.byref(p), plane, self._mc_scratch.ptr, self.stream), "mc_count")
+                    else:
+                        L.check(lib.ivx_dev_mc_count_async(ctypes.byref(p), src, self._mc_scratch.ptr, self.stream), "mc_count")
             with self.timer.span("mc_emit"):
                 self._emit(p, src, plane, z0, cap, self.stream)
             L.check(lib.ivx_dev_mc_total_early(ctypes.byref(p), self._mc_scratch.ptr, ctypes.byref(n), self.stream), "mc_total")
@@ -1018,6 +1052,8 @@
         else:
             p, z0 = self._surface_params(from_binary, min_value, max_value, fill_border_holes)
         self._join_prefetch()
+        self._ride.drop()
+        self._ride.surface_counted(p, z0, False)
         src, plane = self._mc_setup(p, z0)
         nt, nv = ctypes.c_int64(0), ctypes.c_int64(0)
         with self.timer.span("mc_count"):
diff --git a/invesalius3_amd/mc_ride.py b/invesalius3_amd/mc_ride.py
--- /dev/null
+++ b/invesalius3_amd/mc_ride.py
@@ -0,0 +1,30 @@
+from __future__ import annotations
+
+
+class RideBook:
+    def __init__(self, enabled: bool = True):
+        self.enabled = bool(enabled)
+        self.armed = None
+        self.note = None
+        self.rides = 0
+        self.taken = 0
+
+    def piece_to_ride(self):
+        return self.armed if self.enabled else None
+
+    def rode(self, version: int):
+        self.note = (self.armed[0], self.armed[1], int(version))
+        self.armed = None
+        self.rides += 1
+
+    def take(self, params, z0: int, version: int) -> bool:
+        n, self.note = self.note, None
+        ok = n is not None and n[0] is params and n[1] == z0 and n[2] == int(version)
+        self.taken += int(ok)
+        return ok
+
+    def drop(self):
+        self.note = None
+
+    def surface_counted(self, params, z0: int, from_plane: bool):
+        self.armed = (params, z0) if (self.enabled and from_plane) else None
```

Measured after the change: 445,600 Mvoxel/s (median of 6 runs). 1.04x the previous value.
